# martius-lab/iCEM

Measured on AMD Instinct MI355X. Metric: traj-steps/sec (N x h), iCEM inner planning loop, higher is better.
Workload: dtype f32 storage; model step 2xfp16 planes (3 products), f32 accumulate

## Files before the change

icem_amd/_lib.py:

```python
from __future__ import annotations

import ctypes as C
import os

os.environ.setdefault("HSA_ENABLE_IPC_MODE_LEGACY", "0")
from typing import Optional

_HERE = os.path.dirname(os.path.abspath(__file__))
_LIB: Optional[C.CDLL] = None

ICEM_F32, ICEM_F64 = 0, 1
COST_MODES = {"sum": 0, "best": 1, "final": 2}
MODEL_LINEAR, MODEL_TANH = 0, 1
(BUF_MEAN, BUF_STD, BUF_LOW, BUF_HIGH, BUF_OBS0, BUF_ACTIONS, BUF_COSTS, BUF_ELITES, BUF_RECORDS,
 BUF_WORKSPACE, BUF_EXECUTED, BUF_BEST_COST, BUF_COUNT) = range(13)

KERNEL_NAMES = ["sample_clip", "rollout_cost", "topk_partial", "local_pack", "merge_refit", "sample_rollout"]

ICEM_E_INVALID, ICEM_E_UNSUPPORTED, ICEM_E_HIP, ICEM_E_NO_DEVICE, ICEM_E_STATE, ICEM_E_RANGE = -1, -2, -3, -4, -5, -6
ERR_NAMES = {-1: "ICEM_E_INVALID", -2: "ICEM_E_UNSUPPORTED", -3: "ICEM_E_HIP", -4: "ICEM_E_NO_DEVICE",
             -5: "ICEM_E_STATE", -6: "ICEM_E_RANGE"}


class IcemError(RuntimeError):
# ... 39 lines not shown
        "mean", "std", "low", "high", "obs0", "actions", "costs", "elites", "records", "workspace",
        "executed", "best_cost", "z_r", "z_i", "z_r_shift", "z_i_shift")]


_VP, _I32, _I64, _U64, _SZ = C.c_void_p, C.c_int32, C.c_int64, C.c_uint64, C.c_size_t
_H = C.c_void_p
SYMBOLS = [
    ("icem_abi_version", C.c_int, []),
    ("icem_build_hash", C.c_char_p, []),
    ("icem_last_error", C.c_char_p, []),
    ("icem_device_count", C.c_int, []),
    ("icem_create", C.c_int, [C.POINTER(IcemConfigC), C.POINTER(_H)]),
    ("icem_destroy", C.c_int, [_H]),
    ("icem_population_sizes", C.c_int, [_H, C.POINTER(_I32)]),
    ("icem_noise_tables_host", C.c_int, [_I32, C.c_double, C.POINTER(C.c_double), C.POINTER(C.c_double)]),
    ("icem_set_model", C.c_int, [_H, _I32, _I32, C.POINTER(C.c_double), C.POINTER(C.c_double)]),
    ("icem_set_cost", C.c_int, [_H, C.POINTER(IcemCostSpecC)]),
    ("icem_rssm_param_elems", _SZ, []),
    ("icem_rssm_rollout_cost", C.c_int, [_I32, _I32, _I32, _VP, _VP, _VP, _VP, _VP]),
    ("icem_rssm_rollout_cost_batch", C.c_int, [_I32, C.POINTER(_I32), _I32, _I32, _VP, _VP, _VP, _VP, _VP]),
    ("icem_get_action", C.c_int, [_H, C.POINTER(IcemPlanBuffersC), _I32, C.POINTER(C.c_double), C.POINTER(C.c_double),
                                  C.POINTER(C.c_double), _VP]),
    ("icem_set_cost_terms", C.c_int, [_H, C.POINTER(IcemCostTermsC)]),
    ("icem_trajectory_cost", C.c_int, [_H, _I32, _I32, _VP, _VP, _I64, _I64, _VP, _VP, _VP]),
    ("icem_sample_clip", C.c_int, [_H, _I32, _I64, _VP, _VP, _VP, _VP, _VP, _VP, _U64, _I32, _I32, _VP, _VP]),
    ("icem_sample_piecewise", C.c_int, [_H, _I32, _I64, _I32, _I64, _VP, _VP, _VP, _VP, _VP]),
    ("icem_philox_normals", C.c_int, [_H, _I32, _I64, _U64, _VP, _VP, _VP]),
    ("icem_rollout_cost", C.c_int, [_H, _I32, _VP, _VP, _VP, _VP, _VP]),
    ("icem_cost_reduce", C.c_int, [_H, _I32, _VP, _VP, _VP]),
    ("icem_topk_workspace_bytes", _SZ, [_H, _I32, _I32]),
    ("icem_topk_sorted", C.c_int, [_H, _I32, _VP, _I32, _VP, _VP, _VP, _VP]),
    ("icem_gather_refit", C.c_int, [_H, _VP, _VP, _I32, _VP, _VP, _VP, _VP]),
    ("icem_update_distribution", C.c_int, [_H, _I32, _VP, _VP, _I32, _VP, _VP, _I32, _VP, _VP, _VP, _VP, _VP, _VP]),
    ("icem_shift", C.c_int, [_H, _VP, _VP, _VP, _VP, _VP]),
    ("icem_reset_distribution", C.c_int, [_H, _VP, _VP, _VP, _VP, _VP]),
    ("icem_plan_buffer_bytes", _SZ, [_H, _I32]),
    ("icem_plan_iter_local", C.c_int, [_H, C.POINTER(IcemPlanBuffersC), _I32, _I32, _VP]),
    ("icem_plan_iter_merge", C.c_int, [_H, C.POINTER(IcemPlanBuffersC), _I32, _I32, _VP]),
    ("icem_plan_step", C.c_int, [_H, C.POINTER(IcemPlanBuffersC), _I32, _VP]),
    ("icem_record_bytes", _SZ, [_H]),
    ("icem_profile_enable", C.c_int, [_H, _I32]),
    ("icem_debug_stamps", C.c_int, [_H, _VP]),
    ("icem_set_merge_deferral", C.c_int, [_H, C.c_int32]),
    ("icem_set_episode", C.c_int, [_H, C.c_uint64]),
    ("icem_exchange_create", C.c_int, [_H, _VP]),
    ("icem_exchange_connect", C.c_int, [_H, _VP, C.POINTER(C.c_void_p)]),
    ("icem_exchange_block", C.c_void_p, [_H]),
    ("icem_exchange_disable", C.c_int, [_H]),
    ("icem_exchange_status", C.c_int, [_H, C.POINTER(C.c_int32), C.POINTER(C.c_int32)]),
    ("icem_plan_step_sharded", C.c_int, [_H, C.POINTER(IcemPlanBuffersC), _I32, _VP]),
    ("icem_exchange_probe", C.c_int, [_H, C.c_int32, _VP, C.POINTER(C.c_double)]),
    ("icem_sample_truncnorm", C.c_int, [_H, C.c_int32, C.c_int64, _VP, _VP, _VP, _VP, _VP, C.c_uint64, _VP, _VP]),
    ("icem_cem_bounds", C.c_int, [_H, C.c_int32, _VP, _VP, _VP, _VP, _VP, _VP, _VP]),
    ("icem_update_distribution_ok", C.c_int, [_H, C.c_int32, C.c_int32]),
    ("icem_rccl_load", C.c_int, [C.c_char_p]),
    ("icem_rccl_library", C.c_char_p, []),
    ("icem_rccl_unique_id", C.c_int, [_VP]),
    ("icem_rccl_connect", C.c_int, [_H, _VP]),
    ("icem_rccl_adopt", C.c_int, [_H, _VP]),
    ("icem_rccl_disconnect", C.c_int, [_H]),
    ("icem_allgather_elites", C.c_int, [_H, _VP, _VP]),
    ("icem_profile_read", C.c_int, [_H, C.POINTER(C.c_double), C.POINTER(C.c_int64), C.POINTER(C.c_int64)]),
    ("icem_rssm_trim", C.c_int, []),
    ("icem_set_wide_exact", C.c_int, [_H, _I32]),
    ("icem_set_wide_arith", C.c_int, [_H, _I32]),
    ("icem_wide_arith", C.c_int, [_H]),
    ("icem_wide_imbalance_log2", C.c_int, [_H]),
    ("icem_wide_model_imbalance_log2", C.c_int, [_I32, _I32, C.POINTER(C.c_double), C.POINTER(C.c_double)]),
    ("icem_set_tile_arith", C.c_int, [_H, _I32]),
    ("icem_tile_arith", C.c_int, [_H]),
    ("icem_set_f64_arith", C.c_int, [_H, _I32]),
    ("icem_f64_arith", C.c_int, [_H]),
    ("icem_profile_overhead", C.c_int, [_VP, _I32, C.c_double, C.POINTER(C.c_double), C.POINTER(C.c_double)]),
    ("icem_plan_step_batch", C.c_int, [C.POINTER(_H), _I32, C.POINTER(IcemPlanBuffersC), _I32, _VP]),
    ("icem_batch_uploads", C.c_int64, [_H]),
    ("icem_plan_step_batch_f64", C.c_int, [C.POINTER(_H), _I32, C.POINTER(IcemPlanBuffersC), _I32, _VP]),
    ("icem_batch_f64_launches", C.c_int64, [_H]),
    ("icem_plan_step_learned_ok", C.c_int, [_H]),
    ("icem_plan_step_learned", C.c_int, [_H, C.POINTER(IcemPlanBuffersC), _VP, _I32, _VP]),
    ("icem_plan_step_learned_batch", C.c_int, [C.POINTER(_H), _I32, C.POINTER(IcemPlanBuffersC), _VP, C.POINTER(_I32), _VP, _VP]),
    ("icem_learned_step_launches", C.c_int64, [_H]),
    ("icem_tile_growth", C.c_double, [_H]),
    ("icem_nonfinite_costs", C.c_int, [_H, C.POINTER(C.c_int64), _VP]),
    ("icem_set_option", C.c_int, [C.c_char_p, C.c_double]),
    ("icem_get_option", C.c_int, [C.c_char_p, C.POINTER(C.c_double)]),
    ("icem_reset_options", C.c_int, []),
    ("icem_option_name", C.c_char_p, [_I32]),
]


IPC_HANDLE_BYTES = 64
RCCL_ID_BYTES = 128
RSSM_OBS_DIM = 230
ABI_VERSION = 6


def lib_path() -> str:
    return os.environ.get("ICEM_HIP_LIB", os.path.join(_HERE, "libicem_hip.so"))


def load_library() -> C.CDLL:
    global _LIB
    if _LIB is not None:
        return _LIB
    path = lib_path()
    if not os.path.exists(path):
        raise ImportError(f"{path} not found: build it first (python -c 'import __graft_entry__ as g; g.build()'"
                          f" or python -m icem_amd.build)")
    lib = C.CDLL(path)
    for name, res, args in SYMBOLS:
        fn = getattr(lib, name)
        fn.restype = res
        fn.argtypes = args
    if lib.icem_abi_version() != ABI_VERSION:
        raise ImportError(f"{path}: ABI version {lib.icem_abi_version()} != {ABI_VERSION}: rebuild (python -m icem_amd.build)")
    _LIB = lib
    return lib


def option_names():
    lib = load_library()
    out, i = [], 0
    while True:
        n = lib.icem_option_name(i)
        if n is None:
            return out
        out.append(n.decode())
        i += 1


def set_option(name: str, value: float):
    check(load_library().icem_set_option(name.encode(), float(value)))


def get_option(name: str) -> float:
    v = C.c_double()
    check(load_library().icem_get_option(name.encode(), C.byref(v)))
    return v.value


def reset_options():
    check(load_library().icem_reset_options())


_ENV_WORDS = {"thread": 0.0, "rows": 1.0}


def apply_env_options(environ=None) -> dict:
    environ = os.environ if environ is None else environ
    done = {}
    for name in option_names():
        key = "ICEM_" + name.upper()
        if key in environ and environ[key] != "":
            raw = environ[key]
            val = _ENV_WORDS[raw] if raw in _ENV_WORDS else float(raw)
            set_option(name, val)
            done[name] = val
    if environ.get("ICEM_GK_ROLLOUT", "") == "thread":
        set_option("gk_rollout_thread", 1.0)
        done["gk_rollout_thread"] = 1.0
    return done


_FOLLOW_ENV = False


def follow_environment(on: bool = True):
    global _FOLLOW_ENV
    _FOLLOW_ENV = bool(on)
    if on:
        reset_options()
        apply_env_options()


def maybe_follow_environment():
    if _FOLLOW_ENV:
        reset_options()
        apply_env_options()


def check(rc: int):
    if rc != 0:
        msg = load_library().icem_last_error()
        raise IcemError(rc, msg.decode() if msg else "")
```

icem_amd/csrc/abi.hip:

```cpp
#include "host_common.h"
#include "cost_terms_dev.h"
#include "icem_rssm.h"

using namespace icem;

namespace {

void psd_scale_host(int h, double beta, std::vector<double>& s, double& sigma) {
    const int F = h / 2 + 1;
    s.resize(F);
    for (int k = 0; k < F; ++k) s[k] = (double)k * (1.0 / (double)h);
    const double fmin = 1.0 / (double)h;
    int ix = 0;
    for (int k = 0; k < F; ++k) ix += s[k] < fmin ? 1 : 0;
    if (ix && ix < F)
        for (int k = 0; k < ix; ++k) s[k] = s[ix];
    for (int k = 0; k < F; ++k) s[k] = std::pow(s[k], -beta / 2.0);
    double acc = 0.0;
    for (int k = 1; k < F; ++k) {
        double w = s[k];
        if (k == F - 1) w *= (1 + (h % 2)) / 2.0;
        acc += w * w;
    }
    sigma = 2.0 * std::sqrt(acc) / (double)h;
// ... 128 lines not shown
                                  "for its recurrence (that launch's costs are NaN); the staging flags were reset, nothing was "
                                  "launched by this call -- call again");
    ICEM_HIP_TRY(e);
    return ICEM_OK;
}

}

__global__ void profile_spin_kernel(long long ticks, long long* ran) {
    long long t0 = wall_clock64(), t = t0;
    for (long long polls = 0; t - t0 < ticks && polls < (1ll << 26); ++polls) t = wall_clock64();
    if (threadIdx.x == 0) *ran = t - t0;
}

extern "C" {

int icem_abi_version(void) { return ICEM_ABI_VERSION; }

#ifndef ICEM_BUILD_HASH
#define ICEM_BUILD_HASH "0000000000000000"
#endif
const char* icem_build_hash(void) {
    static const char tag[] = "ICEM_BUILD_HASH=" ICEM_BUILD_HASH;
    return tag + 16;
}

const char* icem_last_error(void) { return g_err.c_str(); }

int icem_device_count(void) {
    int n = 0;
    if (hipGetDeviceCount(&n) != hipSuccess) return 0;
    return n;
}

int icem_noise_tables_host(int32_t horizon, double beta, double* cr_host, double* ci_host) {
    if (horizon < 2 || !cr_host || !ci_host) return fail(ICEM_E_INVALID, "bad horizon / null output");
    std::vector<double> cr, ci;
    noise_tables(horizon, beta, cr, ci);
    std::memcpy(cr_host, cr.data(), cr.size() * sizeof(double));
    std::memcpy(ci_host, ci.data(), ci.size() * sizeof(double));
    return ICEM_OK;
}

int icem_create(const icem_config* cfg, icem_handle** out) {
    if (!cfg || !out) return fail(ICEM_E_INVALID, "null argument");
    const icem_config& c = *cfg;
    if (c.num_traj < 2) return fail(ICEM_E_INVALID, "At least two trajectories needed!");
    if (c.horizon < 2 || c.horizon > ICEM_MAX_HORIZON) return fail(ICEM_E_UNSUPPORTED, "horizon must be in [2, 64]");
    if (c.act_dim < 1 || c.act_dim > ICEM_MAX_ACT_DIM) return fail(ICEM_E_UNSUPPORTED, "act_dim must be in [1, 64]");
    if (c.num_elites < 1 || c.num_elites > ICEM_MAX_ELITES) return fail(ICEM_E_UNSUPPORTED, "num_elites must be in [1, 64]");
    if (c.opt_iters < 1) return fail(ICEM_E_INVALID, "opt_iters < 1");
    if (c.dtype != ICEM_F32 && c.dtype != ICEM_F64) return fail(ICEM_E_INVALID, "dtype");
    if (c.rng_rounds != 10 && c.rng_rounds != 7) return fail(ICEM_E_INVALID, "rng_rounds must be 10 or 7");
    if (c.world < 1 || c.rank < 0 || c.rank >= c.world) return fail(ICEM_E_INVALID, "rank/world");
    if (c.noise_beta != c.noise_beta) return fail(ICEM_E_INVALID, "noise_beta is NaN");
    if (!(c.factor_decrease >= 1.0)) return fail(ICEM_E_INVALID, "factor_decrease must be >= 1");
    if (c.cost_mode < 0 || c.cost_mode > 2)
        return fail(ICEM_E_UNSUPPORTED, "Implement method to compute cost along trajectory");
    if (icem_device_count() < 1) return fail(ICEM_E_NO_DEVICE, "no HIP device visible");
    icem_handle* h = new icem_handle();
    h->cfg = c;
    h->F = c.horizon / 2 + 1;
    h->HMAX = c.horizon <= 32 ? 32 : 64;
    h->hd = c.horizon * c.act_dim;
    h->tsize = c.dtype == ICEM_F64 ? 8 : 4;
    h->pop = population_sizes(c);
    h->n_reuse = (int)((double)c.num_elites * c.fraction_reused);
    h->n_local_max = 0;
    for (int n_it : h->pop) h->n_local_max = std::max(h->n_local_max, shard_chunk(n_it, c.world));
    h->use_fast = opt_i(OPT_DISABLE_FAST) == 0;
    std::vector<double> cr, ci, W((size_t)c.horizon * h->HMAX, 0.0);
    if (c.noise_beta > 0) {
        noise_tables(c.horizon, c.noise_beta, cr, ci);
        for (int t = 0; t < c.horizon; ++t)
            for (int m = 0; m < c.horizon; ++m)
                W[(size_t)t * h->HMAX + m] = m < h->F ? cr[(size_t)m * c.horizon + t] : ci[(size_t)(m - h->F + 1) * c.horizon + t];
    } else {
        for (int t = 0; t < c.horizon; ++t) W[(size_t)t * h->HMAX + t] = 1.0;
    }
    int rc = c.dtype == ICEM_F64 ? upload<double>(&h->W_dev, W) : upload<float>(&h->W_dev, W);
    if (!rc && (hipMalloc((void**)&h->nonfinite_dev, 2 * sizeof(unsigned)) != hipSuccess ||
                hipMemset(h->nonfinite_dev, 0, 2 * sizeof(unsigned)) != hipSuccess))
        rc = fail(ICEM_E_HIP, "hipMalloc of the handle's status word failed");
    if (rc) {
        if (h->W_dev) (void)hipFree(h->W_dev);
        if (h->nonfinite_dev) (void)hipFree(h->nonfinite_dev);
        delete h;
        return rc;
    }
    *out = h;
    return ICEM_OK;
}

int icem_destroy(icem_handle* h) {
    if (!h) return ICEM_OK;
    xchg_destroy(h);
    rccl_release(h);
    ahead_destroy(h);
    if (h->W_dev) (void)hipFree(h->W_dev);
    if (h->nonfinite_dev) (void)hipFree(h->nonfinite_dev);
    if (h->actions_alt) (void)hipFree(h->actions_alt);
    if (h->host_stage) (void)hipHostFree(h->host_stage);
    if (h->ws_alt) (void)hipFree(h->ws_alt);
    if (h->pp_stats) (void)hipFree(h->pp_stats);
    if (h->A_dev) (void)hipFree(h->A_dev);
    if (h->B_dev) (void)hipFree(h->B_dev);
    if (h->Mp_dev) (void)hipFree(h->Mp_dev);
    if (h->Mw_dev) (void)hipFree(h->Mw_dev);
    if (h->Mws_dev) (void)hipFree(h->Mws_dev);
    if (h->Mwh_dev) (void)hipFree(h->Mwh_dev);
    if (h->Mwh_ksc_dev) (void)hipFree(h->Mwh_ksc_dev);
    if (h->wide_cs_dev) (void)hipFree(h->wide_cs_dev);
    if (h->M64_dev) (void)hipFree(h->M64_dev);
    if (h->f64_cs_dev) (void)hipFree(h->f64_cs_dev);
    if (h->hn_cs_dev) (void)hipFree(h->hn_cs_dev);
    if (h->pub_dev) (void)hipFree(h->pub_dev);
    if (h->perm_dev) (void)hipFree(h->perm_dev);
    for (auto& sp : h->spans) {
        (void)hipEventDestroy(sp.a);
        (void)hipEventDestroy(sp.b);
    }
    for (auto e : h->free_events) (void)hipEventDestroy(e);
    delete h;
    return ICEM_OK;
}

int icem_set_episode(icem_handle* h, uint64_t episode) {
    if (check_handle(h)) return ICEM_E_INVALID;
    if (episode >> 32) return fail(ICEM_E_INVALID, "episode must fit 32 bits");
    h->episode = episode;
    return ICEM_OK;
}

int icem_population_sizes(const icem_handle* h, int32_t* out_host) {
    if (!h || !out_host) return fail(ICEM_E_INVALID, "null argument");
    for (size_t i = 0; i < h->pop.size(); ++i) out_host[i] = h->pop[i];
    return ICEM_OK;
}

static void update_paths(icem_handle* h) {
    const bool tile = !h->wide && h->has_model && !h->has_terms && !(h->has_cost && h->cost.lin_weight == 0.0) &&
                      fast_rollout_supported(h->cfg.horizon, h->cfg.act_dim, h->O, 1);
    const int of = tile ? h->O : 0;
    if (of != h->Of) h->fast_model_ready = false;
    h->Of = of;
    bool split_ok = of >= 16 && of <= 20 && h->cfg.dtype == ICEM_F32 && !(h->cost.flip_idx >= 0 && h->cost.flip_thresh < 0.0);
    auto lift = [](const std::vector<double>& m, bool* finite) {
        double mx = 0.0;
        for (double v : m) {
            mx = std::max(mx, std::fabs(v));
            if (!(std::fabs(v) < 1e30)) *finite = false;
        }
        if (!(mx > 1e-30)) return 1.f;
        int e = 0;
        (void)std::frexp(mx, &e);
        return (float)std::ldexp(1.0, 7 - e);
    };
    bool finite = true;
    h->tile_m_scale = lift(h->A_host, &finite);
    h->tile_b_scale = lift(h->B_host, &finite);
    const bool narrow_f32 = !h->wide && h->has_model && h->cfg.dtype == ICEM_F32 && finite;
    const bool hn_shape = h->has_model && h->cfg.dtype == ICEM_F32 && finite && h->obs_dim <= 48;
    h->tile_growth = 1.0;
    h->tile_ratio_log2 = 0;
    if ((narrow_f32 || hn_shape) && !h->A_host.empty()) {
        if (h->model_kind == ICEM_MODEL_LINEAR)
            h->tile_growth = linear_growth_bound(h->obs_dim, h->cfg.act_dim, h->cfg.horizon, h->A_host, h->B_host);
        int ea = 0, eb = 0;
        (void)std::frexp((double)h->tile_m_scale, &ea);
        (void)std::frexp((double)h->tile_b_scale, &eb);
        double bmax = 0.0;
        for (double v : h->B_host) bmax = std::max(bmax, std::fabs(v));
        h->tile_ratio_log2 = bmax > 1e-30 ? ea - eb : 0;
    }
    const bool range_ok = finite && h->tile_growth <= 1024.0 && h->tile_ratio_log2 <= 10;
    split_ok = split_ok && range_ok;
    const int mode = h->tile_arith_mode;
    const bool want = mode == 1 || mode < 0;
    h->tile_arith = (split_ok && want) ? 1 : 0;
    int n32 = 0, n4 = 0, np = 0;
    bool terms_ok = true;
    if (h->has_terms && (h->terms.diff_idx >= 0 || h->terms.health_idx >= 0)) terms_ok = false;
    if (h->has_terms)
// ... 1 lines not shown
            const icem_cost_term& tm = h->terms.terms[j];
            if (tm.kind == ICEM_TERM_STEP_GT || tm.kind == ICEM_TERM_SQ_OFFSET) ++np;
            else if (tm.len <= 4) ++n4;
            else if (tm.len <= 32) ++n32;
            else terms_ok = false;
        }
    int prog[3] = {0, 0, 0};
    const bool hn = of == 0 && h->has_model && h->has_cost && h->cfg.dtype == ICEM_F32 && range_ok && mode != 0 && terms_ok &&
                    !(h->wide && h->wide_mode == ICEM_WIDE_F32) &&
                    hn_cost_program(n32, n4, np, prog) &&
                    hn_rollout_supported(h->cfg.horizon, h->cfg.act_dim, h->obs_dim, h->cfg.num_elites);
    for (int k = 0; k < 3; ++k) h->hn_prog[k] = hn ? prog[k] : 0;
    if (hn != h->hn_tile) h->fast_model_ready = false;
    h->hn_tile = hn;
    int eff = 0;
    if (h->wide && h->has_model) {
        eff = h->wide_mode >= 0 ? h->wide_mode : (h->wide_imbalance > 13 ? 2 : 0);
        if (!wide_split_fits(h->obs_dim, h->cfg.act_dim)) eff = 1;
    } else if (gemm_rollout(h)) {
        eff = 1;
    }
    if (eff != h->wide_eff) h->fast_model_ready = false;
    h->wide_eff = eff;
}

static int sync_wide_cost(icem_handle* h);
static int sync_f64_mfma(icem_handle* h);

int icem_set_tile_arith(icem_handle* h, int32_t mode) {
    if (check_handle(h)) return ICEM_E_INVALID;
    if (mode < -1 || mode > 1) return fail(ICEM_E_INVALID, "tile arithmetic: -1 (by configuration), 0 (exact f32) or 1 (fp16 planes)");
    if (h->ride.merge_pending || h->ride.pack_pending) return fail(ICEM_E_STATE, "a deferred merge is pending: finish the MPC step first");
    h->tile_arith_mode = mode;
    update_paths(h);
    h->ahead.next_valid = h->ahead.pre_valid = false;
    return sync_wide_cost(h);
}

int icem_tile_arith(const icem_handle* h) { return h ? ((h->tile_arith || h->hn_tile) ? 1 : 0) : 0; }

double icem_tile_growth(const icem_handle* h) { return h ? h->tile_growth : 0.0; }

int icem_set_option(const char* name, double value) {
    if (!name || !(value == value)) return fail(ICEM_E_INVALID, "null option name / NaN value");
    for (int k = 0; k < OPT_COUNT; ++k)
        if (std::strcmp(name, OPT_ROWS[k].name) == 0) {
            g_opt[k].store(value, std::memory_order_relaxed);
            return ICEM_OK;
        }
    return fail(ICEM_E_INVALID, std::string("unknown option: ") + name);
}

int icem_get_option(const char* name, double* value_out) {
    if (!name || !value_out) return fail(ICEM_E_INVALID, "null argument");
    for (int k = 0; k < OPT_COUNT; ++k)
        if (std::strcmp(name, OPT_ROWS[k].name) == 0) {
            *value_out = g_opt[k].load(std::memory_order_relaxed);
            return ICEM_OK;
        }
    return fail(ICEM_E_INVALID, std::string("unknown option: ") + name);
}

int icem_reset_options(void) {
    for (int k = 0; k < OPT_COUNT; ++k) g_opt[k].store(OPT_ROWS[k].def, std::memory_order_relaxed);
    return ICEM_OK;
}

const char* icem_option_name(int32_t index) { return (index >= 0 && index < OPT_COUNT) ? OPT_ROWS[index].name : nullptr; }

int icem_nonfinite_costs(icem_handle* h, int64_t* count_out, void* stream) {
    if (check_handle(h)) return ICEM_E_INVALID;
    if (!count_out) return fail(ICEM_E_INVALID, "null output");
    hipStream_t st = (hipStream_t)stream;
    hipStreamCaptureStatus cap = hipStreamCaptureStatusNone;
    if (hipStreamIsCapturing(st, &cap) == hipSuccess && cap != hipStreamCaptureStatusNone)
        return fail(ICEM_E_STATE, "icem_nonfinite_costs synchronises: not on a capturing stream");
    unsigned v = 0;
    ICEM_HIP_TRY(hipMemcpyAsync(&v, h->nonfinite_dev, sizeof(v), hipMemcpyDeviceToHost, st));
    ICEM_HIP_TRY(hipStreamSynchronize(st));
    *count_out = (int64_t)v;
    return ICEM_OK;
}

int icem_set_model(icem_handle* h, int32_t kind, int32_t obs_dim, const double* A_host, const double* B_host) {
    if (!h || !A_host || !B_host) return fail(ICEM_E_INVALID, "null argument");
    if (kind != ICEM_MODEL_LINEAR && kind != ICEM_MODEL_TANH) return fail(ICEM_E_INVALID, "model kind");
    const int d = h->cfg.act_dim;
    if (obs_dim > 32 && h->cfg.dtype == ICEM_F64 && h->f64_arith == ICEM_F64_MFMA) {
        if (obs_dim > ICEM_MAX_OBS_DIM || f64_mfma_lds_bytes(obs_dim, d) > 160 * 1024)
            return fail(ICEM_E_UNSUPPORTED, "obs_dim must be in [1, 384]");
        if (h->A_dev) (void)hipFree(h->A_dev);
        if (h->B_dev) (void)hipFree(h->B_dev);
        h->A_dev = h->B_dev = nullptr;
        h->model_kind = kind;
        h->obs_dim = obs_dim;
        h->O = 0;
        h->wide = false;
        h->has_model = true;
        h->A_host.assign(A_host, A_host + (size_t)obs_dim * obs_dim);
        h->B_host.assign(B_host, B_host + (size_t)d * obs_dim);
        h->fast_model_ready = false;
        h->f64_model_ready = false;
        update_paths(h);
        return sync_wide_cost(h);
    }
    if (obs_dim > 32) {
        if (h->cfg.dtype != ICEM_F32 || !wide_rollout_supported(obs_dim, d, 1))
            return fail(ICEM_E_UNSUPPORTED, "obs_dim in (32, 384] needs dtype f32 (k_rollout_wide) or, on an f64 handle, "
                                            "icem_set_f64_arith(ICEM_F64_MFMA); beyond 384 is not compiled");
        if (h->cfg.num_elites > 32) return fail(ICEM_E_UNSUPPORTED, "obs_dim > 32 needs num_elites <= 32 (candidate lists of k_rollout_wide)");
        if (h->A_dev) (void)hipFree(h->A_dev);
        if (h->B_dev) (void)hipFree(h->B_dev);
        h->A_dev = h->B_dev = nullptr;
        h->model_kind = kind;
        h->obs_dim = obs_dim;
        h->O = 0;
        h->wide = true;
        h->has_model = true;
        h->A_host.assign(A_host, A_host + (size_t)obs_dim * obs_dim);
        h->B_host.assign(B_host, B_host + (size_t)d * obs_dim);
        h->wide_imbalance = wide_model_imbalance_log2(obs_dim, d, h->A_host.data(), h->B_host.data());
        h->fast_model_ready = false;
        update_paths(h);
        return sync_wide_cost(h);
    }
    const int O = pick_O(obs_dim);
    if (obs_dim < 1 || O < 0) return fail(ICEM_E_UNSUPPORTED, "obs_dim must be in [1, 384]");
    h->wide = false;
    std::vector<double> A((size_t)O * O, 0.0), B((size_t)d * O, 0.0);
    for (int k = 0; k < obs_dim; ++k)
        for (int i = 0; i < obs_dim; ++i) A[(size_t)k * O + i] = A_host[(size_t)k * obs_dim + i];
    for (int j = 0; j < d; ++j)
        for (int i = 0; i < obs_dim; ++i) B[(size_t)j * O + i] = B_host[(size_t)j * obs_dim + i];
    int rc = h->cfg.dtype == ICEM_F64 ? upload<double>(&h->A_dev, A) : upload<float>(&h->A_dev, A);
    if (rc) return rc;
    rc = h->cfg.dtype == ICEM_F64 ? upload<double>(&h->B_dev, B) : upload<float>(&h->B_dev, B);
    if (rc) return rc;
    h->model_kind = kind;
    h->obs_dim = obs_dim;
    h->O = O;
    h->has_model = true;
    h->A_host.assign(A_host, A_host + (size_t)obs_dim * obs_dim);
    h->B_host.assign(B_host, B_host + (size_t)d * obs_dim);
    h->fast_model_ready = false;
    h->f64_model_ready = false;
    update_paths(h);
    return sync_wide_cost(h);
}

static int sync_f64_mfma(icem_handle* h) {
    if (h->cfg.dtype != ICEM_F64 || h->f64_arith != ICEM_F64_MFMA) return ICEM_OK;
    if (h->has_model && !h->f64_model_ready) {
        const int o = h->obs_dim, d = h->cfg.act_dim, Op = (o + 15) & ~15, Kp = (o + d + 3) & ~3;
        std::vector<double> M((size_t)Kp * Op, 0.0);
        for (int k = 0; k < o; ++k)
            for (int i = 0; i < o; ++i) M[(size_t)k * Op + i] = h->A_host[(size_t)k * o + i];
        for (int j = 0; j < d; ++j)
            for (int i = 0; i < o; ++i) M[(size_t)(o + j) * Op + i] = h->B_host[(size_t)j * o + i];
        const int rc = upload<double>(&h->M64_dev, M);
        if (rc) return rc;
        h->f64_model_ready = true;
    }
    if (h->has_cost) {
        CostArgs<double> cs;
        std::memset((void*)&cs, 0, sizeof(cs));
        fill_cost_args_f64(h, cs);
// ... 367 lines not shown
```

icem_amd/csrc/fused_dev.h:

```cpp
#pragma once
#include "icem_fused.h"

#include <climits>
#include <cmath>
#include <cstdlib>
#include <algorithm>
#include <type_traits>
#include <utility>

#include "exchange_dev.h"
#include "philox.h"
#include "refit.h"

#ifndef ICEM_FAST_SHAPES
#define ICEM_FAST_SHAPES(X) X(30, 6, 17) X(30, 6, 18) X(12, 6, 17) X(13, 4, 17) X(30, 17, 24)
#endif
#define ICEM_FAST_HORIZONS(X) X(30) X(12) X(13) X(10)

namespace icem {

namespace {

constexpr int HMAX = 32;
constexpr int SWG = 256;
// ... 886 lines not shown
        use_min = a.cost_mode == 1;
        flip_th = a.flip_th;
    }
    __device__ __forceinline__ void load_obs(const float* obs) {
        x_init = obs[perm_c];
#pragma unroll
        for (int r = 0; r < REM; ++r) rem_init[r] = obs[perm_rem[r]];
    }
    __device__ __forceinline__ const float* read_ptr(const float* buf, int row, int stride) const {
        return buf + T16::SLACK + row * stride + (g - REM);
    }
    __device__ __forceinline__ const float* row_ptr(const float* buf, int row, int stride) const {
        return buf + T16::SLACK + row * stride;
    }
    struct State {
        float x;
        float xr[REM > 0 ? REM : 1];
        float acc_s, acc_b;
    };
    __device__ __forceinline__ void init(State& st) const {
        st.x = x_init;
#pragma unroll
        for (int r = 0; r < REM; ++r) st.xr[r] = rem_init[r];
        st.acc_s = 0.f;
        st.acc_b = INFINITY;
    }
    __device__ __forceinline__ void step(State& st, const float* rd, const float* ar) const {
        float xv[NKX];
#pragma unroll
        for (int q = 0; q < NKX; ++q) {
            const float ld = rd[4 * q];
            float v = is_act[q] ? ld : 0.f;
#pragma unroll
            for (int r = 0; r < REM; ++r)
                if (r / 4 == q) v = (g == r % 4) ? st.xr[r] : v;
            xv[q] = v;
        }
        float ext[NE];
#pragma unroll
        for (int e = 0; e < NE; ++e) ext[e] = e < REM ? st.xr[e] : (e - REM < D ? ar[e - REM] : 0.f);
        const float col0 = dpp_f32<0x00>(st.x);
        const float col1 = dpp_f32<0x55>(st.x);
        const float ang = ang_is_col1 ? col1 : col0;
        float cst = 0.f;
        cst += (ang > flip_th) ? pen : 0.f;
        cst += (ang < -flip_th) ? pen : 0.f;
#pragma unroll
        for (int q = 0; q < NKX; ++q) cst = __builtin_fmaf(xv[q] * xv[q], cw[q], cst);
        cst = __builtin_fmaf(lin_w, col0, cst);
        float pr[REM > 0 ? REM : 1];
        if (REM > 0) {
            const float col2 = dpp_f32<0xAA>(st.x), col3 = dpp_f32<0xFF>(st.x);
            const float cq[4] = {col0, col1, col2, col3};
#pragma unroll
            for (int r = 0; r < REM; ++r) {
                float p = 0.f;
#pragma unroll
                for (int s = 0; s < 4; ++s) p = __builtin_fmaf(cq[s], wq[r][s], p);
#pragma unroll
                for (int q = 0; q < NKX; ++q) p = __builtin_fmaf(xv[q], wx[r][q], p);
                pr[r] = reduce_quads(p);
            }
        }
        cst = reduce_quads(cst);
        st.acc_s = __builtin_fmaf(st.acc_s, ksum, cst);
        st.acc_b = cst < st.acc_b ? cst : st.acc_b;
        float nxt = 0.f;
        asm volatile("s_nop 1" ::: "memory");
#define ICEM_T4(K) nxt = fmac_row_bcast<K>(nxt, st.x, mK[K]);
        ICEM_T4(0) ICEM_T4(4) ICEM_T4(8) ICEM_T4(12)
        ICEM_T4(1) ICEM_T4(5) ICEM_T4(9) ICEM_T4(13)
        ICEM_T4(2) ICEM_T4(6) ICEM_T4(10) ICEM_T4(14)
        ICEM_T4(3) ICEM_T4(7) ICEM_T4(11) ICEM_T4(15)
#undef ICEM_T4
#pragma unroll
        for (int e = 0; e < NE; ++e) nxt = __builtin_fmaf(mE[e], ext[e], nxt);
        st.x = act_fn(nxt, std::integral_constant<int, KIND>{});
#pragma unroll
        for (int r = 0; r < REM; ++r) st.xr[r] = act_fn(pr[r], std::integral_constant<int, KIND>{});
    }
    __device__ __forceinline__ float cost(const State& st) const { return use_min ? st.acc_b : st.acc_s; }
};

template <bool LANE_MASK = true>
__device__ __forceinline__ unsigned long long topk_push16(unsigned long long run_key, unsigned long long key, bool first,
                                                          int K, int lane) {
    if (!first) {
        const unsigned long long prev = __shfl(run_key, lane - 16, 64);
        if (lane >= 16 && lane < 16 + K) key = prev;
    }
    return wave_sort_n<LANE_MASK>(key, lane, first ? 16u : 16u + (unsigned)K);
}

constexpr unsigned KEY_FILL_LO = 0x7FFFFE00u;
template <int WAVES>
__device__ __forceinline__ void wg_merge_emit(unsigned long long (*wg_keys)[WAVES][32], unsigned long long run_key, int K,
                                              int lane, int wave, const FastRolloutArgs& a, int wg = blockIdx.x,
                                              int n_wg = gridDim.x) {
    static_assert(WAVES * 32 <= 512, "filler keys: one per slot");
    auto emit = [&](unsigned long long key, int place) {
        if (a.part_k) {
            a.part_k[(size_t)place * n_wg + wg] = key;
        } else {
            a.part_c[(size_t)wg * K + place] = key_cost(key);
            a.part_i[(size_t)wg * K + place] = key_idx(key);
        }
    };
    if (WAVES == 1) {
        if (wave == 0 && lane < K) emit(run_key, lane);
        return;
    }
    const int kp = (K + 1) & ~1, half = kp >> 1;
    unsigned long long* keys = &wg_keys[0][0][0];
    if (wave < WAVES && lane < kp) {
        unsigned long long v = lane < K ? run_key : KEY_SENTINEL;
        if (v == KEY_SENTINEL) v = (KEY_SENTINEL & 0xFFFFFFFF00000000ull) | (KEY_FILL_LO + (unsigned)(wave * 32 + lane));
        keys[wave * 32 + lane] = v;
    }
    __syncthreads();
    if (wave < WAVES) {
        const int q = lane >> 4;
        for (int s0 = 0; s0 < K; s0 += 16) {
            const int i = s0 + (lane & 15);
            const unsigned long long mine = keys[wave * 32 + (i < 32 ? i : 31)];
            unsigned place = 0;
            for (int r = q; r < WAVES; r += 4) {
                const unsigned long long* b = keys + r * 32;
#pragma unroll 4
                for (int c = 0; c < half; ++c) place += (b[2 * c] < mine ? 1u : 0u) + (b[2 * c + 1] < mine ? 1u : 0u);
            }
            place += (unsigned)__shfl_xor((int)place, 16, 64);
            place += (unsigned)__shfl_xor((int)place, 32, 64);
            if (q == 0 && i < K && place < (unsigned)K) {
                const bool filler = (mine >> 32) == (KEY_SENTINEL >> 32) && (unsigned)mine >= KEY_FILL_LO;
                emit(filler ? KEY_SENTINEL : mine, (int)place);
            }
        }
    }
}

constexpr int MERGE_WG = 256;
constexpr int LPL = 4;

template <int CTRL, int ROW_MASK>
__device__ __forceinline__ unsigned long long min_dpp(unsigned long long x) {
    const int lo = __builtin_amdgcn_update_dpp((int)(unsigned)x, (int)(unsigned)x, CTRL, ROW_MASK, 0xF, false);
    const int hi = __builtin_amdgcn_update_dpp((int)(unsigned)(x >> 32), (int)(unsigned)(x >> 32), CTRL, ROW_MASK, 0xF, false);
    const unsigned long long o = ((unsigned long long)(unsigned)hi << 32) | (unsigned)lo;
    return o < x ? o : x;
}

__device__ __forceinline__ unsigned long long wave_min_u64(unsigned long long x) {
    x = min_dpp<0xB1, 0xF>(x);
    x = min_dpp<0x4E, 0xF>(x);
    x = min_dpp<0x141, 0xF>(x);
    x = min_dpp<0x140, 0xF>(x);
    x = min_dpp<0x142, 0xA>(x);
    x = min_dpp<0x143, 0xC>(x);
    const unsigned lo = __builtin_amdgcn_readlane((int)(unsigned)x, 63);
    const unsigned hi = __builtin_amdgcn_readlane((int)(unsigned)(x >> 32), 63);
    return ((unsigned long long)hi << 32) | lo;
}

template <int CTRL, int ROW_MASK>
__device__ __forceinline__ unsigned min_dpp32(unsigned x) {
    const unsigned o = (unsigned)__builtin_amdgcn_update_dpp((int)x, (int)x, CTRL, ROW_MASK, 0xF, false);
    return o < x ? o : x;
}
__device__ __forceinline__ unsigned wave_min_u32(unsigned x) {
    x = min_dpp32<0xB1, 0xF>(x);
    x = min_dpp32<0x4E, 0xF>(x);
    x = min_dpp32<0x141, 0xF>(x);
    x = min_dpp32<0x140, 0xF>(x);
    x = min_dpp32<0x142, 0xA>(x);
    x = min_dpp32<0x143, 0xC>(x);
    return (unsigned)__builtin_amdgcn_readlane((int)x, 63);
}
__device__ __forceinline__ unsigned long long wave_min_key(unsigned long long x) {
    const unsigned hi = (unsigned)(x >> 32), lo = (unsigned)x;
    const unsigned mh = wave_min_u32(hi);
    const unsigned long long tie = __ballot(hi == mh);
    unsigned ml;
    if (__popcll(tie) == 1)
        ml = (unsigned)__builtin_amdgcn_readlane((int)lo, __ffsll((long long)tie) - 1);
    else
        ml = wave_min_u32(hi == mh ? lo : 0xFFFFFFFFu);
    return ((unsigned long long)mh << 32) | ml;
}

template <int CTRL, int ROW_MASK>
__device__ __forceinline__ unsigned add_dpp(unsigned x) {
    return x + (unsigned)__builtin_amdgcn_update_dpp(0, (int)x, CTRL, ROW_MASK, 0xF, ROW_MASK == 0xF);
}
__device__ __forceinline__ unsigned wave_incl_scan_u32(unsigned x) {
    x = add_dpp<0x111, 0xF>(x);
    x = add_dpp<0x112, 0xF>(x);
    x = add_dpp<0x114, 0xF>(x);
    x = add_dpp<0x118, 0xF>(x);
    x = add_dpp<0x142, 0xA>(x);
    x = add_dpp<0x143, 0xC>(x);
    return x;
}

__device__ __forceinline__ unsigned long long lds_reread_u64(const unsigned long long* p) {
#ifdef ICEM_DEBUG
    if (!__builtin_amdgcn_is_shared(p)) __builtin_trap();
#endif
    return *(const volatile __attribute__((address_space(3))) unsigned long long*)p;
}

__device__ __forceinline__ int keep_index0(const MergeSingleArgs& a) { return a.keep_base >= 0 ? a.keep_base : a.n_global; }

__device__ __forceinline__ float merge_keep_cost(const MergeSingleArgs& a, int lane) {
    const bool has = a.elites_cost_cur != nullptr;
    const float* src = has ? a.elites_cost_cur : reinterpret_cast<const float*>(a.part_k);
    const float v = src[(has && lane < a.n_keep) ? lane : 0];
    return has ? v : 0.f;
}

template <int KREG>
__device__ __forceinline__ void merge_select(const MergeSingleArgs& a, int lane, unsigned long long* cand,
                                             unsigned long long* sel) {
    unsigned long long k[LPL][KREG];
    const float keep_cost = merge_keep_cost(a, lane);
#pragma unroll
    for (int l = 0; l < LPL; ++l) {
        const int list = lane + l * 64;
#pragma unroll
        for (int i = 0; i < KREG; ++i)
            k[l][i] = a.part_k[(size_t)(i < a.K ? i : 0) * a.n_lists + (list < a.n_lists ? list : 0)];
    }
#pragma unroll
    for (int l = 0; l < LPL; ++l) {
        const bool has_list = lane + l * 64 < a.n_lists;
#pragma unroll
        for (int i = 0; i < KREG; ++i) k[l][i] = (has_list && i < a.K) ? k[l][i] : KEY_SENTINEL;
    }
    if (a.dbg && threadIdx.x == 0) a.dbg[1] = wall_clock64();
    if (lane < a.n_keep) {
        unsigned long long v = make_key(keep_cost, keep_index0(a) + lane);
#pragma unroll
        for (int i = 0; i < KREG; ++i) {
            const bool sw = v < k[0][i];
            const unsigned long long t = sw ? k[0][i] : v;
            k[0][i] = sw ? v : k[0][i];
            v = t;
        }
    }
    if (a.dbg && threadIdx.x == 0) a.dbg[2] = wall_clock64();
    unsigned long long mine = k[0][0];
#pragma unroll
    for (int l = 1; l < LPL; ++l) mine = k[l][0] < mine ? k[l][0] : mine;
    const unsigned srt = wave_sort64_u32((unsigned)(mine >> 32), lane);
    const unsigned T = __shfl(srt, a.K - 1, 64);
    unsigned n_cand = 0;
#pragma unroll
    for (int i = 0; i < KREG; ++i) {
        bool p[LPL];
        bool any_lane = false;
#pragma unroll
        for (int l = 0; l < LPL; ++l) {
            p[l] = (unsigned)(k[l][i] >> 32) <= T && k[l][i] != KEY_SENTINEL;
            any_lane |= p[l];
        }
        if (__ballot(any_lane) == 0) break;
#pragma unroll
        for (int l = 0; l < LPL; ++l) {
            const unsigned long long m = __ballot(p[l]);
            if (m != 0) {
                const unsigned pos = n_cand + __builtin_amdgcn_mbcnt_hi((unsigned)(m >> 32), __builtin_amdgcn_mbcnt_lo((unsigned)m, 0u));
                if (p[l] && pos < 64) cand[pos] = k[l][i];
                n_cand += (unsigned)__popcll(m);
            }
        }
    }
    if (a.dbg && threadIdx.x == 0) a.dbg[3] = wall_clock64();
    __builtin_amdgcn_fence(__ATOMIC_SEQ_CST, "workgroup");
    if (n_cand <= 64) {
        unsigned long long key = lane < (int)n_cand ? lds_reread_u64(&cand[lane]) : KEY_SENTINEL;
        key = wave_sort_n(key, lane, n_cand);
        if (lane < a.K) sel[lane] = key;
    } else {
        for (int r = 0; r < a.K; ++r) {
            unsigned long long head = k[0][0];
#pragma unroll
            for (int l = 1; l < LPL; ++l) head = k[l][0] < head ? k[l][0] : head;
            const unsigned long long best = wave_min_u64(head);
            if (best != KEY_SENTINEL) {
#pragma unroll
                for (int l = 0; l < LPL; ++l) {
                    if (k[l][0] == best) {
#pragma unroll
                        for (int i = 0; i + 1 < KREG; ++i) k[l][i] = k[l][i + 1];
                        k[l][KREG - 1] = KEY_SENTINEL;
                    }
                }
            }
            if (lane == 0) sel[r] = best;
        }
    }
}

__device__ __forceinline__ void merge_select_stream(const MergeSingleArgs& a, int lane, unsigned long long* cand,
                                                    unsigned long long* sel) {
    const int K = a.K, nl = a.n_lists;
    auto key_at = [&](int l, int i) -> unsigned long long {
        const int list = lane + l * 64;
        const unsigned long long v = a.part_k[(size_t)(i < K ? i : 0) * nl + (list < nl ? list : 0)];
        return (list < nl && i < K) ? v : KEY_SENTINEL;
    };
    const unsigned long long kept = lane < a.n_keep ? make_key(a.elites_cost_cur[lane], keep_index0(a) + lane) : KEY_SENTINEL;
    unsigned long long mine = kept;
#pragma unroll
    for (int l = 0; l < LPL; ++l) {
        const unsigned long long v = key_at(l, 0);
        mine = v < mine ? v : mine;
    }
    const unsigned long long srt = wave_sort64(mine, lane);
    const unsigned long long T = __shfl(srt, K - 1, 64);
    unsigned n_cand = 0;
    auto offer = [&](unsigned long long key) {
        const bool p = key <= T && key != KEY_SENTINEL;
        const unsigned long long m = __ballot(p);
        if (m != 0) {
            const unsigned pos = n_cand + __builtin_amdgcn_mbcnt_hi((unsigned)(m >> 32), __builtin_amdgcn_mbcnt_lo((unsigned)m, 0u));
            if (p && pos < 64) cand[pos] = key;
            n_cand += (unsigned)__popcll(m);
        }
        return m != 0;
    };
    offer(kept);
#pragma unroll 1
    for (int l = 0; l < LPL; ++l) {
        if (l * 64 >= nl) break;
#pragma unroll 1
        for (int i = 0; i < K; ++i)
            if (!offer(key_at(l, i))) break;
    }
    __builtin_amdgcn_fence(__ATOMIC_SEQ_CST, "workgroup");
    if (n_cand <= 64) {
        unsigned long long key = lane < (int)n_cand ? lds_reread_u64(&cand[lane]) : KEY_SENTINEL;
        key = wave_sort_n(key, lane, n_cand);
        if (lane < K) sel[lane] = key;
    } else {
        int cur[LPL];
#pragma unroll
        for (int l = 0; l < LPL; ++l) cur[l] = 0;
        bool kept_live = true;
        for (int r = 0; r < K; ++r) {
            unsigned long long head = kept_live ? kept : KEY_SENTINEL;
#pragma unroll
            for (int l = 0; l < LPL; ++l) {
                const unsigned long long v = key_at(l, cur[l]);
                head = v < head ? v : head;
            }
            const unsigned long long best = wave_min_u64(head);
            if (best != KEY_SENTINEL) {
                if (kept_live && kept == best) kept_live = false;
#pragma unroll
                for (int l = 0; l < LPL; ++l)
                    if (key_at(l, cur[l]) == best) ++cur[l];
            }
            if (lane == 0) sel[r] = best;
        }
    }
}

template <int DEPTH>
__device__ __forceinline__ void merge_select_shallow(const MergeSingleArgs& a, int lane, unsigned long long* cand,
                                                     unsigned long long* sel) {
    const int K = a.K, nl = a.n_lists;
    const float keep_cost = merge_keep_cost(a, lane);
    unsigned long long k[LPL][DEPTH];
#pragma unroll
    for (int l = 0; l < LPL; ++l) {
        const int list = lane + l * 64;
#pragma unroll
        for (int i = 0; i < DEPTH; ++i) k[l][i] = a.part_k[(size_t)(i < K ? i : 0) * nl + (list < nl ? list : 0)];
    }
#pragma unroll
    for (int l = 0; l < LPL; ++l) {
        const bool has_list = lane + l * 64 < nl;
#pragma unroll
        for (int i = 0; i < DEPTH; ++i) k[l][i] = (has_list && i < K) ? k[l][i] : KEY_SENTINEL;
    }
    const unsigned long long kept = lane < a.n_keep ? make_key(keep_cost, keep_index0(a) + lane) : KEY_SENTINEL;
    unsigned long long mine = k[0][0];
#pragma unroll
    for (int l = 1; l < LPL; ++l) mine = k[l][0] < mine ? k[l][0] : mine;
    const unsigned srt = wave_sort64_u32((unsigned)(mine >> 32), lane);
    const unsigned T = __shfl(srt, K - 1, 64);
    unsigned n_cand = 0;
    auto offer = [&](unsigned long long key) {
        const bool p = (unsigned)(key >> 32) <= T && key != KEY_SENTINEL;
        const unsigned long long m = __ballot(p);
        if (m != 0) {
            const unsigned pos = n_cand + __builtin_amdgcn_mbcnt_hi((unsigned)(m >> 32), __builtin_amdgcn_mbcnt_lo((unsigned)m, 0u));
            if (p && pos < 64) cand[pos] = key;
            n_cand += (unsigned)__popcll(m);
        }
        return m != 0;
    };
    bool deeper[LPL];
#pragma unroll
    for (int l = 0; l < LPL; ++l) {
        deeper[l] = true;
#pragma unroll
        for (int i = 0; i < DEPTH; ++i)
            if (deeper[l]) deeper[l] = offer(k[l][i]);
    }
#pragma unroll 1
    for (int l = 0; l < LPL; ++l) {
        if (!deeper[l]) continue;
#pragma unroll 1
        for (int i = DEPTH; i < K; ++i) {
            const int list = lane + l * 64;
            const unsigned long long v = list < nl ? a.part_k[(size_t)i * nl + list] : KEY_SENTINEL;
            if (!offer(v)) break;
        }
    }
    offer(kept);
    __builtin_amdgcn_fence(__ATOMIC_SEQ_CST, "workgroup");
    if (n_cand <= 64) {
        unsigned long long key = lane < (int)n_cand ? lds_reread_u64(&cand[lane]) : KEY_SENTINEL;
        key = wave_sort_n(key, lane, n_cand);
        if (lane < K) sel[lane] = key;
    } else {
        merge_select_stream(a, lane, cand, sel);
    }
}

__device__ __forceinline__ void merge_select_records(const MergeSingleArgs& a, int lane, unsigned long long* cand,
                                                     unsigned long long* sel, int* slot, long long* stamp = nullptr) {
    const int K = a.K, rs = a.h * a.d + 2;
    xchg_wait(a.xw, lane);
    if (stamp && lane == 0) *stamp = wall_clock64();
    auto rec_key = [&](int e) -> unsigned long long {
        if (e >= a.n_rec) return KEY_SENTINEL;
        const float* rec = a.records + (size_t)e * rs;
        return make_key(rec[0], reinterpret_cast<const int*>(rec + 1)[0]);
    };
    unsigned long long k[3] = {rec_key(lane), rec_key(lane + 64),
                               lane < a.n_keep ? make_key(a.elites_cost_cur[lane], a.n_global + lane) : KEY_SENTINEL};
    const unsigned long long k0 = k[0], k1 = k[1], k2 = k[2];
    for (int r = 0; r < K; ++r) {
        unsigned long long head = k[0] < k[1] ? k[0] : k[1];
        head = k[2] < head ? k[2] : head;
        const unsigned long long best = wave_min_key(head);
        if (best != KEY_SENTINEL) {
            if (k0 == best) { slot[r] = lane; k[0] = KEY_SENTINEL; }
            if (k1 == best) { slot[r] = lane + 64; k[1] = KEY_SENTINEL; }
            if (k2 == best) { slot[r] = a.n_rec + lane; k[2] = KEY_SENTINEL; }
        } else if (lane == 0) {
            slot[r] = 0;
        }
        if (lane == 0) sel[r] = best;
    }
    (void)cand;
}

__device__ __forceinline__ void merge_select_records_wg(const MergeSingleArgs& a, bool stager, int lane, int tid, int nthr,
                                                        unsigned long long* sel, int* slot, long long* stamp = nullptr) {
    __shared__ unsigned long long rk_keys[192];
    __shared__ unsigned rk_rank[192];
    const int K = a.K, rs = a.h * a.d + 2;
    if (stager) {
        xchg_wait(a.xw, lane);
        if (stamp && lane == 0) *stamp = wall_clock64();
        auto rec_key = [&](int e) -> unsigned long long {
            if (e >= a.n_rec) return KEY_SENTINEL;
            const float* rec = a.records + (size_t)e * rs;
            return make_key(rec[0], reinterpret_cast<const int*>(rec + 1)[0]);
        };
        rk_keys[lane] = rec_key(lane);
        rk_keys[64 + lane] = rec_key(lane + 64);
        rk_keys[128 + lane] = lane < a.n_keep ? make_key(a.elites_cost_cur[lane], a.n_global + lane) : KEY_SENTINEL;
        rk_rank[lane] = rk_rank[64 + lane] = rk_rank[128 + lane] = 0u;
        sel[lane] = KEY_SENTINEL;
        slot[lane] = 0;
    }
    __syncthreads();
    const int n_rec = a.n_rec, n_live = n_rec + a.n_keep;
    auto at = [&](int c) { return c < n_rec ? c : 128 + (c - n_rec); };
    int parts = n_live > 0 ? nthr / n_live : 1;
    parts = parts < 1 ? 1 : (parts > 8 ? 8 : parts);
    if (n_live > 0 && tid < n_live * parts) {
        const int c = tid % n_live, p = tid / n_live;
        const unsigned long long mine = rk_keys[at(c)];
        unsigned cnt = 0;
        for (int j = p; j < n_live; j += parts) cnt += rk_keys[at(j)] < mine ? 1u : 0u;
        if (cnt) atomicAdd(&rk_rank[at(c)], cnt);
    }
    if (n_live > nthr)
        for (int c = nthr + tid; c < n_live; c += nthr) {
            const unsigned long long mine = rk_keys[at(c)];
            unsigned cnt = 0;
            for (int j = 0; j < n_live; ++j) cnt += rk_keys[at(j)] < mine ? 1u : 0u;
            rk_rank[at(c)] = cnt;
        }
    __syncthreads();
    for (int c = tid; c < n_live; c += nthr) {
        const unsigned long long mine = rk_keys[at(c)];
        const unsigned r = rk_rank[at(c)];
        if (mine != KEY_SENTINEL && r < (unsigned)K) {
            sel[r] = mine;
            slot[r] = c;
        }
    }
    __syncthreads();
}

// ... 477 lines not shown
```

icem_amd/csrc/host_common.h:

```cpp
#pragma once
#include <hip/hip_runtime.h>

#include <cfloat>
#include <climits>
#include <cmath>
#include <cstdio>
#include <cstdlib>
#include <cstring>
#include <algorithm>
#include <atomic>
#include <string>
#include <type_traits>
#include <vector>

#include "../../include/icem_hip.h"
#include "arg_array.h"
#include "icem_fused.h"
#include "options.h"

namespace icem {

inline thread_local std::string g_err;

inline int fail(int code, const std::string& msg) {
    g_err = msg;
    return code;
}

#define ICEM_HIP_TRY(expr)                                                                      \
    do {                                                                                        \
        hipError_t e_ = (expr);                                                                 \
        if (e_ != hipSuccess)                                                                   \
            return ::icem::fail(ICEM_E_HIP, std::string(#expr) + ": " + hipGetErrorString(e_)); \
    } while (0)

constexpr int WG = 256;
constexpr int TOPK_CHUNK = 1024;

struct Exchange;

struct LearnedCtx {
    DeviceArgArray<2> args;
    float* pool = nullptr;
    size_t pool_rows = 0;
    int pool_n = 0;
    int* idx = nullptr;
    long long launches = 0;
    ~LearnedCtx() {
        if (pool) (void)hipFree(pool);
        if (idx) (void)hipFree(idx);
    }
};

}

struct icem_handle {
    icem_config cfg;
    int F = 0, HMAX = 0, hd = 0;
    size_t tsize = 4;
    void* W_dev = nullptr;
    int model_kind = 0, obs_dim = 0, O = 0;
    void* A_dev = nullptr;
    void* B_dev = nullptr;
    bool has_model = false, has_cost = false;
    icem_cost_spec cost;
    icem_cost_terms terms;
    bool has_terms = false;
    void* host_stage = nullptr;
    void* host_stage_dev = nullptr;
    unsigned io_seq = 0;
    std::vector<int> pop;
    int n_reuse = 0;
    int n_local_max = 0;
    bool profiling = false;
    struct Span {
        int kind;
        long long units;
        hipEvent_t a, b;
    };
    bool use_fast = true;
    long long* dbg = nullptr;
    struct LocalReport {
        int lists = 0;
        int tail_rows = 0;
        int sel_cand = 0, sel_loc = 0;
        void clear() { *this = LocalReport(); }
    } local;
    void* actions_alt = nullptr;
    void* ws_alt = nullptr;
    float* pp_stats = nullptr;
    struct Riding {
        bool merge_pending = false;
        icem::MergeSingleArgs merge;
        bool pack_pending = false;
        icem::PackPrev pack;
        void clear() { merge_pending = pack_pending = false; }
    } ride;
    bool deferral = false;
    float* cur_mean = nullptr;
    float* cur_std = nullptr;
    bool wide = false;
    int Of = 0;
    int tile_arith_mode = -1;
    int tile_arith = 0;
    int hn_prog[3] = {0, 0, 0};
    void* hn_cs_dev = nullptr;
    bool hn_tile = false;
    float tile_m_scale = 1.f, tile_b_scale = 1.f;
    float act_mag = 1.f;
    const void* am_lo = nullptr;
    const void* am_hi = nullptr;
    double tile_growth = 1.0;
    int tile_ratio_log2 = 0;
    unsigned* nonfinite_dev = nullptr;
    unsigned nonfinite_seen = 0;
    void* Mw_dev = nullptr;
    void* Mws_dev = nullptr;
    void* Mwh_dev = nullptr;
    float Mwh_inv = 1.f;
    void* Mwh_ksc_dev = nullptr;
    int Mwh_nk = 0;
    float Mwh_sbound = 0.f;
    int wide_mode = -1;
    int wide_eff = 0;
    int wide_imbalance = 0;
    int wide_packed = -2;
    void* wide_cs_dev = nullptr;
    int f64_arith = 0;
    void* M64_dev = nullptr;
    bool f64_model_ready = false;
    void* f64_cs_dev = nullptr;
    void* Mp_dev = nullptr;
    void* perm_dev = nullptr;
    int flip_col = -1;
    bool fast_model_ready = false;
    std::vector<double> A_host, B_host;
    std::vector<Span> spans;
    std::vector<hipEvent_t> free_events;
    icem::Exchange* xchg = nullptr;
    icem::XchgWait xw_last;
    uint64_t episode = 0;
    float* pub_dev = nullptr;
    unsigned pub_seq = 0;
    struct Ahead {
        void* pool[3] = {nullptr, nullptr, nullptr};
        unsigned long long ctr = 0;
        bool next_valid = false;
        uint64_t next_episode = 0;
        int next_step = -1;
        void* next_pool = nullptr;
        hipStream_t next_stream = nullptr;
        const void* lo_ptr = nullptr;
        const void* hi_ptr = nullptr;
        bool uniform = false;
        float lo = 0.f, hi = 0.f;
        bool tail_pending = false;
        icem::FastSampleArgs tail_args, tail2_args;
        int next1_rows = 0;
        void* next1_pool = nullptr;
        void* pre_raw = nullptr;
        bool pre_valid = false;
        uint64_t pre_episode = 0;
        int pre_step = -1;
        hipStream_t pre_stream = nullptr;
        int disabled = -1;
        int min_rows = 0;
    } ahead;
    icem::DeviceArgArray<6> batch_args;
    unsigned long long batch_uploads = 0;
    long long batch_f64_launches = 0;
    icem::LearnedCtx learned;
    void* rccl_comm = nullptr;
    bool rccl_owned = false;
};

namespace icem {

struct ProfScope {
    icem_handle* h;
    hipStream_t st;
    hipEvent_t a = nullptr, b = nullptr;
    int kind;
    long long units;
    static hipEvent_t get(icem_handle* h) {
        if (!h->free_events.empty()) {
            hipEvent_t e = h->free_events.back();
            h->free_events.pop_back();
            return e;
        }
        hipEvent_t e = nullptr;
        (void)hipEventCreate(&e);
        return e;
    }
    ProfScope(const icem_handle* hc, int kind_, long long units_, hipStream_t st_)
        : h(const_cast<icem_handle*>(hc)), st(st_), kind(kind_), units(units_) {
        if (!h->profiling) return;
        a = get(h);
        b = get(h);
// ... 151 lines not shown
```

icem_amd/csrc/icem_fused.h:

```cpp
#pragma once
#include <hip/hip_runtime.h>
#include <stdint.h>
#include <cstddef>
#include <cstring>
#include <vector>
#include "cost_args.h"
#include "options.h"

namespace icem {

constexpr int FAST_MAX_LISTS = 256;
struct BatchHint;
struct LaunchCtx;

constexpr int XCHG_MAX_WORLD = 16;
struct XchgWait {
    const unsigned* flags = nullptr;
    unsigned* status = nullptr;
    unsigned seq = 0;
    int world = 0;
    unsigned max_polls = 0;
    const void* records = nullptr;
};
struct XchgPush {
// ... 160 lines not shown
    const float* keep_actions;
    int n, n_keep, K, hd;
    float alpha;
    float* mean;
    float* std;
    float* elites_out;
    float* elite_costs_out;
    int* idx_out;
};
void launch_update_small(const UpdateSmallArgs& a, hipStream_t st);
constexpr int UPDATE_FINISH_MAX_HD = 256;
struct UpdateFinishArgs {
    UpdateSmallArgs u;
    int d;
    float init_std;
    const float* low;
    const float* high;
    float* executed;
    float* best_cost;
    float* result;
};
void launch_update_small_batch(const UpdateFinishArgs* args_dev, int n, bool finish, hipStream_t st);
bool topk_small_ok(int n, int K);
void launch_topk_small(const float* costs, int n, int K, float* out_c, int* out_i, hipStream_t st);
bool pack_can_push(int K, int h, int d);
void launch_pack_records(const MergeSingleArgs& a, int n_loc, int shard_lo, float* records, hipStream_t st,
                         const XchgPush& px = XchgPush());
void launch_pack_merge(const MergeSingleArgs& pk, int n_loc, int shard_lo, float* records, const XchgPush& px, const MergeSingleArgs& m,
                       hipStream_t st);

struct PackPrev {
    const unsigned long long* part_k = nullptr;
    const float* actions = nullptr;
    int n_lists = 0, n_pool = 0, n_global = 0, K = 0;
    int n_loc = 0, shard_lo = 0;
    int n_keep = 0;
    const float* keep_costs = nullptr;
    float* records = nullptr;
    XchgPush px;
    float* pub = nullptr;
    unsigned* pub_flag = nullptr;
    unsigned pub_seq = 0;
};
bool sample_rollout_pack_ok(const BatchHint& bh, int h, int d, int O, int rounds, int n_rows, int K);
bool sample_folded_pack_ok(int h, int d, int rounds, int K);

void launch_noise_rows(const FastSampleArgs& a, int rounds, hipStream_t st);
struct IterAheadArgs {
    FastRolloutArgs r;
    MergeSingleArgs m;
    int has_merge;
    int n_xf;
    int row0_mean;
    int store_back;
    float* pool;
    const float* mean;
    const float* std;
    float lo, hi;
    FastSampleArgs z;
    FastSampleArgs s;
    PackPrev p;
    int n_roll, n_noise;
    int dbg_slot = 0;
};
bool rollout_ahead_ok(const BatchHint& bh, int h, int d, int O, int K, int n_rows);
int ahead_roll_workgroups(const BatchHint& bh, int n_rows);
void launch_iter_ahead(const LaunchCtx& cx, const IterAheadArgs& a, int h, int d, int O, int kind);

struct FastSampleMergeArgs {
    FastSampleArgs s;
    MergeSingleArgs m;
    PackPrev p;
};
bool sample_folded_merge_ok(int h, int d, int rounds, int K);
void launch_sample_folded_merge(const LaunchCtx& cx, const FastSampleMergeArgs& a);
bool sample_batch_compiled(int h);

struct FastIterArgs {
    FastSampleArgs s;
    FastRolloutArgs r;
    MergeSingleArgs m;
    PackPrev p;
};
}
#include "generic_args.h"
namespace icem {
constexpr int ICEM_MAX_BATCH = 32;
struct BatchBases {
    unsigned long long v[ICEM_MAX_BATCH];
};
struct BatchHint {
    int mult = 1;
    bool ahead = false;
};
enum LaunchFamily : int { LAUNCH_SAMPLE_ROLLOUT = 1, LAUNCH_ITER_AHEAD = 2, LAUNCH_MERGE_NOISE = 3, LAUNCH_SAMPLE = 4, LAUNCH_SAMPLE_MERGE = 5,
                          LAUNCH_ROLLOUT_HN = 6, LAUNCH_GK_SAMPLE = 7, LAUNCH_GK_SHIFT = 8, LAUNCH_GK_ROLLOUT_ROWS = 9, LAUNCH_GK_ROLLOUT_THREAD = 10,
                          LAUNCH_GK_SELECT = 11, LAUNCH_ROLLOUT_WIDE = 12, LAUNCH_ROLLOUT_WIDE_SPLIT = 13, LAUNCH_ROLLOUT_ROWS_WIDE = 14 };
struct LaunchKey {
    int family = 0;
    int h = 0, d = 0, O = 0, kind = 0, arith = 0;
    int waves = 0;
    int form = 0;
    int wgs[3] = {0, 0, 0};
    bool operator==(const LaunchKey& o) const { return std::memcmp(this, &o, sizeof(LaunchKey)) == 0; }
};
struct MergeNoiseBatchArgs {
    MergeSingleArgs a;
    FastSampleArgs z1, z2;
};
struct LaunchDesc {
    LaunchKey key;
    static constexpr size_t BLOCK = sizeof(IterAheadArgs) > sizeof(RolloutArgs<double>) ? sizeof(IterAheadArgs) : sizeof(RolloutArgs<double>);
    static_assert(sizeof(SelectArgs<double>) <= BLOCK && sizeof(SampleArgs<double>) <= BLOCK, "LaunchDesc::block");
    alignas(8) unsigned char block[BLOCK];
};
struct LaunchRecorder {
    unsigned long long base = 0;
    std::vector<LaunchDesc> launches;
    bool unsupported = false;
    const char* who = "icem_plan_step_batch: ";
    void* add(const LaunchKey& key) {
        launches.emplace_back();
        launches.back().key = key;
        std::memset(launches.back().block, 0, sizeof(launches.back().block));
        return launches.back().block;
    }
};
struct LaunchCtx {
    hipStream_t st = nullptr;
    BatchHint hint;
    LaunchRecorder* rec = nullptr;
};
template <class Form, class Issue>
void submit(const LaunchCtx& cx, const LaunchKey& key, bool batched_form, Form&& form, Issue&& issue) {
    if (!cx.rec) return issue();
    if (!batched_form) cx.rec->unsupported = true;
    else form(cx.rec->add(key), cx.rec->base);
}
inline void sub_base(uint32_t& lo, uint32_t& hi, unsigned long long base) {
    const unsigned long long v = (((unsigned long long)hi << 32) | lo) - base;
    lo = (uint32_t)v;
    hi = (uint32_t)(v >> 32);
}
inline void batch_form(const FastIterArgs& a, unsigned long long base, void* dst) {
    std::memcpy(dst, &a, sizeof(a));
    FastSampleArgs& s = ((FastIterArgs*)dst)->s;
    if (s.n_shift == 0) s.off2_lo = s.off2_hi = 0;
    else sub_base(s.off2_lo, s.off2_hi, base);
    sub_base(s.off_lo, s.off_hi, base);
}
inline void batch_form(const IterAheadArgs& a, unsigned long long base, void* dst) {
    constexpr size_t defined = offsetof(IterAheadArgs, dbg_slot) + sizeof(int);
    std::memcpy(dst, &a, defined);
    IterAheadArgs& g = *(IterAheadArgs*)dst;
    g.r.dbg = nullptr;
    if (g.z.n > 0) sub_base(g.z.off_lo, g.z.off_hi, base);
    else g.z.off_lo = g.z.off_hi = 0;
    if (g.s.n_shift > 0) {
        sub_base(g.s.off_lo, g.s.off_hi, base);
        sub_base(g.s.off2_lo, g.s.off2_hi, base);
    } else {
        g.s.off_lo = g.s.off_hi = g.s.off2_lo = g.s.off2_hi = 0;
    }
}
inline void batch_form(const MergeSingleArgs& a, const FastSampleArgs* z1, const FastSampleArgs* z2, unsigned long long base, void* dst) {
    MergeNoiseBatchArgs& g = *(MergeNoiseBatchArgs*)dst;
// ... 139 lines not shown
```

icem_amd/csrc/k_iter_small.hip:

```cpp
#include "fused_dev.h"

namespace icem {

namespace {

constexpr bool sr_quad(int d, int rw) { return rw <= 2 && ((4 * 16 * rw * d + 63) / 64) * 64 + 64 <= 1024; }
constexpr int sr_threads(int d, int rw) { return (((sr_quad(d, rw) ? 4 : 1) * 16 * rw * d + 63) / 64) * 64; }

template <int H, int D, int O, int KIND, int ROUNDS, int RW, int KREG, bool REC, int ARITH>
__device__ __forceinline__ void sample_rollout_body(const FastSampleArgs& sa, const FastRolloutArgs& ra, const MergeSingleArgs& am,
                                                    const PackPrev& ap) {
    constexpr bool PM = KREG > 0;
    constexpr bool QS = sr_quad(D, RW);
    constexpr bool T4 = QS && O <= 20 && sr_threads(D, RW) >= 256 * RW && ARITH == 0;
    using T16 = typename TileSel<H, D, O, KIND, ARITH>::type;
    using Tile = typename std::conditional<T4, Tile4<H, D, (O <= 20 ? O : 17), KIND>, T16>::type;
    constexpr int RWV = T4 ? 4 * RW : RW;
    constexpr int HD = H * D;
    constexpr int TPB = 16 * RW;
    constexpr int ROWS = TPB * D;
    constexpr int NT = sr_threads(D, RW);
    constexpr int NTT = NT + (PM ? 64 : 0);
    static_assert(NTT <= 1024 && HD % 2 == 0, "workgroup shape");
    constexpr int VW = HD % 4 == 0 ? 4 : 2;
    using Vec = typename VecOf<VW>::type;
    __shared__ __attribute__((aligned(16))) float ms[2 * HD];
    __shared__ __attribute__((aligned(16))) float tilebuf[T16::SLACK + TPB * HD + T16::TAIL];
    __shared__ unsigned long long wg_keys[2][RW][32];
    __shared__ float obs_stage[32];
    constexpr int WROWS = H / 2 + 1;
    __shared__ __attribute__((aligned(16))) float Wl[QS ? NT / 64 : 1][QS ? WROWS * WQ_STRIDE : 4];
    __shared__ unsigned long long sel[PM ? 64 : 1];
    __shared__ unsigned long long cand[PM ? 64 : 1];
    __shared__ int slot[PM ? 64 : 1];
    float* tile_rows = tilebuf + T16::SLACK;
    const int tid = threadIdx.x;
    const int lane = tid & 63;
    const int wave = tid >> 6;
    const int n_rows = ra.n_rows;
    const bool has_pack = PM && REC && ap.part_k != nullptr;
    if constexpr (PM && REC) {
        if (has_pack && blockIdx.x == 0) {
            MergeSingleArgs pk{};
            pk.n_lists = ap.n_lists;
            pk.n_pool = ap.n_pool;
            pk.n_global = ap.n_global;
            pk.K = ap.K;
            pk.h = H;
            pk.d = D;
            pk.part_k = ap.part_k;
            pk.actions = ap.actions;
            pk.n_keep = ap.n_keep;
            pk.elites_cost_cur = ap.keep_costs;
            pk.keep_base = ap.n_loc;
            __builtin_amdgcn_s_setprio(3);
            if (ra.dbg && tid == 0) ra.dbg[0] = wall_clock64();
            if (tid < 64) {
                if constexpr (NTT <= 512)
                    merge_select<12>(pk, lane, cand, sel);
                else
                    merge_select_stream(pk, lane, cand, sel);
            }
            __syncthreads();
            if (ra.dbg && tid == 0) ra.dbg[1] = wall_clock64();
            pack_records_body<12>(pk, ap.n_loc, ap.shard_lo, ap.records, ap.px, tilebuf, sel, tid, NTT);
            if (ra.dbg && tid == 0) ra.dbg[2] = wall_clock64();
            return;
        }
    }
    const int wg = blockIdx.x - (has_pack ? 1 : 0);
    const int n_wg = ra.list_wgs > 0 ? ra.list_wgs : (int)gridDim.x - (has_pack ? 1 : 0);
    const int base = wg * TPB;
    if (base >= n_rows) return;
    if (ra.dbg && tid == 0 && wg == 0) ra.dbg[8] = wall_clock64();
    const int rowi = QS ? tid >> 2 : tid, q = tid & 3;
    const int nl = rowi / D, jd = rowi - nl * D;
    const bool has_row = rowi < ROWS;
    float* trow = tile_rows + nl * HD + jd;
    const float* mrow = ms + jd;
    Tile tile;
    float obs_reg = 0.f;
    constexpr int WPL = (WROWS * HMAX + 63) / 64;
    float wreg[QS ? WPL : 1];
    const bool pre_drawn = !PM && sa.raw_src != nullptr;
    if constexpr (QS) {
        if (tid < NT && !pre_drawn) {
#pragma unroll
            for (int i = 0; i < WPL; ++i) wreg[i] = sa.W[(i * 64 + lane) < WROWS * HMAX ? i * 64 + lane : 0];
        }
    }
    const int r_mine = base + nl;
    float lo_reg = 0.f, hi_reg = 0.f;
    if ((PM || pre_drawn) && tid < NT) {
        lo_reg = sa.low[jd];
        hi_reg = sa.high[jd];
    }
    constexpr int NVR = !PM ? (TPB * (HD / VW) + NTT - 1) / NTT : 1;
    constexpr int NVB = NVR < 4 ? NVR : 4;
    constexpr int NEL = !PM && QS ? (H - 1 + 3) / 4 : 1;
    typedef float RawV __attribute__((ext_vector_type(VW)));
    RawV rawv[NVB];
    float elv[NEL];
    if (!PM) {
        const int total4 = (n_rows - base < TPB ? n_rows - base : TPB) * (HD / VW);
        RawV* t4 = reinterpret_cast<RawV*>(tile_rows);
        float mreg[(HD + NTT - 1) / NTT], sreg[(HD + NTT - 1) / NTT];
#pragma unroll
        for (int i = 0; i < (HD + NTT - 1) / NTT; ++i) {
            const int e = tid + i * NTT;
            mreg[i] = sa.mean[e < HD ? e : 0];
            sreg[i] = sa.std[e < HD ? e : 0];
        }
        if (pre_drawn) {
            const RawV* g4 = reinterpret_cast<const RawV*>(sa.raw_src + (size_t)base * HD);
#pragma unroll
            for (int i = 0; i < NVB; ++i) {
                const int e = tid + i * NTT;
                rawv[i] = g4[e < total4 ? e : 0];
            }
            if constexpr (QS) {
                if (has_row && tid < NT && r_mine >= sa.n && r_mine < n_rows) {
                    const float* src = sa.elites_src + (size_t)(r_mine - sa.n) * HD + jd;
#pragma unroll
                    for (int i = 0; i < NEL; ++i) elv[i] = src[(q + 4 * i < H - 1 ? q + 4 * i + 1 : 1) * D];
                }
            }
        }
        obs_reg = ra.obs0[(tid < 32 && tid < ra.o) ? tid : 0];
        if (wave < RWV) tile.load(ra, lane);
#pragma unroll
        for (int i = 0; i < (HD + NTT - 1) / NTT; ++i) {
            const int e = tid + i * NTT;
            if (e < HD) {
                ms[e] = mreg[i];
                ms[HD + e] = sreg[i];
            }
        }
        if (pre_drawn) {
#pragma unroll
            for (int i = 0; i < NVB; ++i) {
                const int e = tid + i * NTT;
                if (e < total4) t4[e] = rawv[i];
            }
            if constexpr (NVR > NVB) {
                const RawV* g4 = reinterpret_cast<const RawV*>(sa.raw_src + (size_t)base * HD);
                for (int e0 = tid + NVB * NTT; e0 < total4; e0 += NVB * NTT) {
#pragma unroll
                    for (int i = 0; i < NVB; ++i) rawv[i] = g4[e0 + i * NTT < total4 ? e0 + i * NTT : 0];
#pragma unroll
                    for (int i = 0; i < NVB; ++i)
                        if (e0 + i * NTT < total4) t4[e0 + i * NTT] = rawv[i];
                }
            }
        }
// ... 4 lines not shown
        if (has_row && tid < NT) {
            const float lo = lo_reg, hi = hi_reg;
            constexpr int QN = QS ? 4 : 1;
            const int q0 = QS ? q : 0;
            if (r_mine < sa.n) {
                for (int t = q0; t < H; t += QN) {
                    const float v = __builtin_fmaf(trow[t * D], mrow[HD + t * D], mrow[t * D]);
                    trow[t * D] = __builtin_amdgcn_fmed3f(v, lo, hi);
                }
            } else if (r_mine < n_rows) {
                const float* src = sa.elites_src + (size_t)(r_mine - sa.n) * HD + jd;
                if ((H - 1) % QN == q0) {
                    const float v = __builtin_fmaf(trow[(H - 1) * D], mrow[HD + (H - 1) * D], mrow[(H - 1) * D]);
                    trow[(H - 1) * D] = __builtin_amdgcn_fmed3f(v, lo, hi);
                }
                if constexpr (QS) {
#pragma unroll
                    for (int i = 0; i < NEL; ++i)
                        if (q + 4 * i < H - 1) trow[(q + 4 * i) * D] = elv[i];
                } else {
                    for (int t = q0; t < H - 1; t += QN) trow[t * D] = src[(t + 1) * D];
                }
            } else {
                for (int t = q0; t < H; t += QN) trow[t * D] = 0.f;
            }
        }
    } else
    if constexpr (QS) {
        if (tid < NT) {
            float* wl = Wl[wave];
            sample_into_tile_quad<H, D, ROUNDS, PM>(sa, has_row, n_rows, r_mine, jd, q, trow, mrow, wl, [&]() {
#pragma unroll
                for (int i = 0; i < WPL; ++i) {
                    const int e = i * 64 + lane;
                    if (e < WROWS * HMAX) wl[(e / HMAX) * WQ_STRIDE + (e % HMAX)] = wreg[i];
                }
                __builtin_amdgcn_fence(__ATOMIC_RELEASE, "wavefront");
                __builtin_amdgcn_wave_barrier();
                __builtin_amdgcn_fence(__ATOMIC_ACQUIRE, "wavefront");
            });
        }
    } else if (has_row) {
        sample_into_tile<H, D, ROUNDS, PM>(sa, n_rows, r_mine, jd, trow, mrow);
    }
    if constexpr (PM) {
        if (tid >= NT) {
            if constexpr (RW <= 4) __builtin_amdgcn_s_setprio(3);
            if constexpr (REC) {
                if (ra.dbg && lane == 0 && wg == 0) ra.dbg[3] = wall_clock64();
            }
            else if constexpr (RW >= 8)
                merge_select_stream(am, lane, cand, sel);
            else
                merge_select_shallow<3>(am, lane, cand, sel);
        }
    }
    if (PM) {
        obs_reg = ra.obs0[(tid < 32 && tid < ra.o) ? tid : 0];
        if (wave < RWV) tile.load(ra, lane);
    }
    const float* rd0 = nullptr;
    if constexpr (!T4) rd0 = tile.read_ptr(tilebuf + (wave < RW ? wave : 0) * 16 * HD, lane, HD);
    if constexpr (PM) {
        const MergeSingleArgs& m = am;
        if constexpr (REC) {
            merge_select_records_wg(am, tid >= NT, lane, tid, NTT, sel, slot, (ra.dbg && wg == 0) ? ra.dbg + 7 : nullptr);
            if (ra.dbg && tid == 0 && wg == 0) ra.dbg[4] = wall_clock64();
        } else {
            __syncthreads();
        }
        if (ra.dbg && tid == 0 && wg == 0) ra.dbg[5] = wall_clock64();
        if (!REC && ra.dbg && tid == 0 && wg == 0) ra.dbg[15] = wall_clock64();
        const float* rows[KREG > 0 ? KREG : 1];
        merge_rows<KREG, REC>(m, sel, slot, rows);
        for (int e = tid; e < HD; e += NTT) {
            float xs[KREG > 0 ? KREG : 1];
#pragma unroll
            for (int r = 0; r < KREG; ++r) xs[r] = rows[r][e];
            float nm, ns;
            refit_element_regs<float, KREG>(m.K, m.alpha, m.mean[e], m.std[e], xs, nm, ns);
            ms[e] = nm;
            ms[HD + e] = ns;
            if (wg == 0) {
                m.mean_out[e] = nm;
                m.std_out[e] = ns;
#pragma unroll
                for (int r = 0; r < KREG; ++r)
                    if (r < m.K) m.elites_next[(size_t)r * HD + e] = xs[r];
            }
        }
        if (wg == 0 && tid < m.K) m.elites_cost_next[tid] = key_cost(sel[tid]);
        __syncthreads();
        if (ra.dbg && tid == 0 && wg == 0) ra.dbg[6] = wall_clock64();
        if (!REC && ra.dbg && tid == 0 && wg == 0) ra.dbg[7] = wall_clock64();
        if (has_row && r_mine < sa.n) {
            const float lo = lo_reg, hi = hi_reg;
            for (int t = QS ? q : 0; t < H; t += QS ? 4 : 1) {
                const float v = __builtin_fmaf(trow[t * D], mrow[HD + t * D], mrow[t * D]);
                trow[t * D] = __builtin_amdgcn_fmed3f(v, lo, hi);
            }
        }
    }
    if (tid < 32) {
        float ov = obs_reg;
        asm volatile("" : "+v"(ov));
        obs_stage[tid] = tid < ra.o ? ov : 0.f;
    }
    if (ra.dbg && tid == 0 && wg == 0) ra.dbg[10] = wall_clock64();
    __syncthreads();
    if (sa.row0_mean && sa.first_index + base == 0) {
        for (int e = tid; e < HD; e += NTT) tile_rows[e] = ms[e];
        __syncthreads();
    }
    {
        const int total4 = (n_rows - base < TPB ? n_rows - base : TPB) * (HD / VW);
        const Vec* t4 = reinterpret_cast<const Vec*>(tile_rows);
        Vec* g4 = reinterpret_cast<Vec*>(sa.out + (size_t)base * HD);
        constexpr int CP0 = (NTT - 64 * RWV >= 128) ? 64 * RWV : 0;
        if (tid >= CP0)
            for (int e = tid - CP0; e < total4; e += NTT - CP0) g4[e] = t4[e];
    }
    if (ra.dbg && tid == 0 && wg == 0) ra.dbg[11] = wall_clock64();
    unsigned long long run_key = KEY_SENTINEL;
    if constexpr (T4) {
        if (wave < RWV) {
            tile.load_obs(obs_stage);
            const int rs = wave * 4 + (lane >> 4);
            const int row = base + rs;
            const float* rd = tile.read_ptr(tilebuf, rs, HD);
            const float* ar = tile.row_ptr(tilebuf, rs, HD);
            typename Tile::State st;
            tile.init(st);
#pragma unroll
            for (int t = 0; t < H; ++t) tile.step(st, rd + t * D, ar + t * D);
            const float cost = tile.cost(st);
            const bool live = row < n_rows;
            if ((lane & 15) == 0) {
                if (live) ra.costs[row] = cost;
                note_nonfinite(ra, cost, live);
                wg_keys[0][0][rs] = (live && row < ra.n_cand) ? make_key(cost, row)
                                    : TPB <= 16 ? KEY_SENTINEL : ((KEY_SENTINEL & 0xFFFFFFFF00000000ull) | (KEY_FILL_LO + (unsigned)rs));
            }
        }
        if (ra.dbg && tid == 0 && wg == 0) ra.dbg[13] = wall_clock64();
        if (ra.K > 0 && wg < n_wg) {
            __syncthreads();
            if (wave == 0 && TPB <= 16) {
                const unsigned long long key = wave_sort_first<16>(lane < TPB ? wg_keys[0][0][lane] : KEY_SENTINEL, lane);
                if (lane < ra.K) {
                    if (ra.part_k) {
                        ra.part_k[(size_t)lane * n_wg + wg] = key;
                    } else {
                        ra.part_c[(size_t)wg * ra.K + lane] = key_cost(key);
                        ra.part_i[(size_t)wg * ra.K + lane] = key_idx(key);
                    }
                }
            } else if (wave == 0) {
                constexpr int NK = TPB <= 16 ? 16 : 32, PARTS = 64 / NK, PER = NK / PARTS;
                static_assert(TPB <= 32 && PER % 2 == 0, "one wave counts for the slab");
                const unsigned long long* keys = &wg_keys[0][0][0];
                const int i = lane & (NK - 1), part = lane / NK;
                const unsigned long long mine = i < TPB ? keys[i] : KEY_SENTINEL;
                unsigned place = 0;
#pragma unroll
                for (int c = 0; c < PER; ++c) {
                    const int e = part * PER + c;
                    place += (e < TPB && keys[e < TPB ? e : 0] < mine) ? 1u : 0u;
                }
                if (NK == 16) place += (unsigned)__shfl_xor((int)place, 16, 64);
                place += (unsigned)__shfl_xor((int)place, 32, 64);
                if (part == 0 && i < TPB && place < (unsigned)ra.K) {
                    const bool filler = (mine >> 32) == (KEY_SENTINEL >> 32) && (unsigned)mine >= KEY_FILL_LO;
                    const unsigned long long key = filler ? KEY_SENTINEL : mine;
                    if (ra.part_k) {
                        ra.part_k[(size_t)place * n_wg + wg] = key;
                    } else {
                        ra.part_c[(size_t)wg * ra.K + place] = key_cost(key);
                        ra.part_i[(size_t)wg * ra.K + place] = key_idx(key);
                    }
                }
            }
        }
    } else {
        if (wave < RW) {
            tile.load_obs(obs_stage);
            run_key = rollout_slab<Tile, H, D, true>(tile, ra, rd0, base + wave * 16 + (lane & 15), n_rows, run_key, true, lane);
            if (ra.dbg && tid == 0 && wg == 0) ra.dbg[12] = wall_clock64();
        }
        if (ra.dbg && tid == 0 && wg == 0) ra.dbg[13] = wall_clock64();
        if (ra.K > 0 && wg < n_wg) wg_merge_emit<RW>(wg_keys, run_key, ra.K, lane, wave, ra, wg, n_wg);
    }
    if (ra.dbg && tid == 0 && wg == 0) ra.dbg[14] = wall_clock64();
}


template <int H, int D, int O, int KIND, int ROUNDS, int RW, int KREG, bool REC, int ARITH>
__global__ __launch_bounds__(sr_threads(D, RW) + (KREG > 0 ? 64 : 0)) void sample_rollout_kernel(FastIterArgs a) {
    sample_rollout_body<H, D, O, KIND, ROUNDS, RW, KREG, REC, ARITH>(a.s, a.r, a.m, a.p);
}

template <int H, int D, int O, int KIND, int ROUNDS, int RW, int KREG, int ARITH>
__global__ __launch_bounds__(sr_threads(D, RW) + (KREG > 0 ? 64 : 0)) void sample_rollout_batch_kernel(const FastIterArgs* __restrict__ args,
                                                                                                      BatchBases bases) {
    const FastIterArgs& a = args[blockIdx.y];
    FastSampleArgs s = from_device(a.s);
    const unsigned long long base = bases.v[blockIdx.y];
    add_base64(s.off_lo, s.off_hi, base);
    add_base64(s.off2_lo, s.off2_hi, base);
    const FastRolloutArgs r = from_device(a.r);
    const MergeSingleArgs m = from_device(a.m);
    sample_rollout_body<H, D, O, KIND, ROUNDS, RW, KREG, false, ARITH>(s, r, m, a.p);
}

}

constexpr int single_launch_max_rw(int h, int d) {
    int best = 0;
    for (int rw = 1; rw <= 8; rw *= 2)
        if (sr_threads(d, rw) + 64 <= 1024 && 16 * rw * h * d * 4 <= 120 * 1024) best = rw;
    return best;
}

static bool sample_rollout_shape(const BatchHint& bh, int h, int d, int O, int rounds, int n_rows, int n_tail, int* grid_out, int* rw_out,
                                 int* tail_out = nullptr) {
    const int max_rw = opt_i(OPT_FUSE_MAX_RW);
    int grid, rw, tail = 0;
    r16_shape(n_rows, &grid, &rw);
    const int mult = bh.mult;
    if (mult > 1) {
        int g_all, rw_all;
        r16_shape(n_rows * mult, &g_all, &rw_all);
        const int cap = opt_i(OPT_BATCH_MAX_RW);
        rw = std::min(std::max(rw, rw_all), std::min(cap > 0 ? cap : 8, single_launch_max_rw(h, d)));
        while (rw > 1 && rw > single_launch_max_rw(h, d)) rw /= 2;
        grid = (std::max(1, (n_rows + 15) / 16) + rw - 1) / rw;
        if (grid > FAST_MAX_LISTS) return false;
    } else
    if (n_tail > 0 && n_tail <= 64) {
        int g2, w2;
        r16_shape(n_rows - n_tail, &g2, &w2);
        if (w2 < rw && sr_threads(d, w2) + 64 <= 512 && g2 == FAST_MAX_LISTS && n_rows - n_tail == FAST_MAX_LISTS * 16 * w2) {
            rw = w2;
            tail = n_tail;
        }
    }
    if (rounds != 10 || rw > max_rw || n_rows <= 0 || !fast_rollout_supported(h, d, O, 1) || !fast_sample_supported(h, d))
        return false;
    if (rw > single_launch_max_rw(h, d)) return false;
    *grid_out = tail ? (n_rows + 16 * rw - 1) / (16 * rw) : std::min(grid, (n_rows + 16 * rw - 1) / (16 * rw));
    *rw_out = rw;
    if (tail_out) *tail_out = tail;
    return true;
}

int sample_rollout_lists(const BatchHint& bh, int h, int d, int O, int rounds, int n_rows, int n_tail, int* tail_out) {
    int grid, rw, tail = 0;
    if (!sample_rollout_shape(bh, h, d, O, rounds, n_rows, n_tail, &grid, &rw, &tail)) return 0;
    if (tail_out) *tail_out = tail;
    return tail ? FAST_MAX_LISTS : grid;
}

bool sample_rollout_merge_ok(const BatchHint& bh, int h, int d, int O, int rounds, int n_rows, int K) {
    const int on = opt_i(OPT_MERGE_PROLOGUE);
    int grid, rw;
    return on && K + 1 <= 12 && sample_rollout_shape(bh, h, d, O, rounds, n_rows, 0, &grid, &rw);
}

bool sample_rollout_pack_ok(const BatchHint& bh, int h, int d, int O, int rounds, int n_rows, int K) {
    const int on = opt_i(OPT_RIDING_PACK);
    int grid, rw;
    return on && sample_rollout_merge_ok(bh, h, d, O, rounds, n_rows, K) && sample_rollout_shape(bh, h, d, O, rounds, n_rows, 0, &grid, &rw) &&
           K * (h * d + 2) <= 16 * rw * h * d;
}

namespace {
template <int H, int D, int O, int KIND, int RW, int KREG, bool REC, int ARITH>
struct SrInst {
    static constexpr int THREADS = sr_threads(D, RW) + (KREG > 0 ? 64 : 0);
    static constexpr bool BATCHED = !REC;
    static void solo(int grid, hipStream_t st, const FastIterArgs& a) {
        hipLaunchKernelGGL((sample_rollout_kernel<H, D, O, KIND, 10, RW, KREG, REC, ARITH>), dim3(grid), dim3(THREADS), 0, st, a);
    }
    static void batch(int grid, int n, hipStream_t st, const FastIterArgs* args_dev, const BatchBases& bases) {
        hipLaunchKernelGGL((sample_rollout_batch_kernel<H, D, O, KIND, 10, RW, KREG, ARITH>), dim3(grid, n), dim3(THREADS), 0, st, args_dev, bases);
    }
};
template <int H, int D, int O, int RW, class F>
bool sample_rollout_pick(const LaunchKey& k, F& f) {
    if constexpr (RW > single_launch_max_rw(H, D)) {
        return false;
    } else {
        if (k.waves != RW) return false;
        auto with = [&](auto kind, auto arith) {
            constexpr int KK = decltype(kind)::value, AA = decltype(arith)::value;
            if (k.form == 2) f(SrInst<H, D, O, KK, RW, 12, true, AA>{});
            else if (k.form == 1) f(SrInst<H, D, O, KK, RW, 12, false, AA>{});
            else f(SrInst<H, D, O, KK, RW, 0, false, AA>{});
            return true;
        };
        using I0 = std::integral_constant<int, 0>;
        using I1 = std::integral_constant<int, 1>;
        if constexpr (O <= 20) {
            if (k.arith == 1) return k.kind == 1 ? with(I1{}, I1{}) : with(I0{}, I1{});
        }
        return k.kind == 1 ? with(I1{}, I0{}) : with(I0{}, I0{});
    }
}
template <class F>
bool sample_rollout_dispatch(const LaunchKey& k, F&& f) {
#define XR(HH, DD, OO)                                                                                      \
    if (k.h == HH && k.d == DD && k.O == OO)                                                                \
        return sample_rollout_pick<HH, DD, OO, 1>(k, f) || sample_rollout_pick<HH, DD, OO, 2>(k, f) ||      \
               sample_rollout_pick<HH, DD, OO, 4>(k, f) || sample_rollout_pick<HH, DD, OO, 8>(k, f);
    ICEM_FAST_SHAPES(XR)
#undef XR
    return false;
}
}

void launch_sample_rollout(const LaunchCtx& cx, const FastIterArgs& a, int h, int d, int O, int kind, bool merge_prologue) {
    LaunchKey k;
    if (!sample_rollout_shape(cx.hint, h, d, O, 10, a.r.n_rows, a.r.list_wgs > 0 ? a.s.n_shift : 0, &k.wgs[0], &k.waves)) return;
    k.family = LAUNCH_SAMPLE_ROLLOUT;
    k.h = h, k.d = d, k.O = O, k.kind = kind, k.arith = a.r.arith;
    k.form = !merge_prologue ? 0 : a.m.records ? 2 : 1;
    k.wgs[1] = (k.form == 2 && a.p.part_k) ? 1 : 0;
    submit(cx, k, k.form != 2, [&](void* dst, unsigned long long base) { batch_form(a, base, dst); },
           [&] { sample_rollout_dispatch(k, [&](auto inst) { inst.solo(k.wgs[0] + k.wgs[1], cx.st, a); }); });
}

void launch_sample_rollout_batch(const LaunchKey& k, const FastIterArgs* args_dev, const BatchBases& bases, int n, hipStream_t st) {
    sample_rollout_dispatch(k, [&](auto inst) {
        if constexpr (decltype(inst)::BATCHED) inst.batch(k.wgs[0], n, st, args_dev, bases);
    });
}

}
```

icem_amd/csrc/k_merge.hip:

```cpp
#include "fused_dev.h"
#include "refit.h"

namespace icem {

namespace {

template <int KREG, bool REC>
__device__ __forceinline__ void merge_single_body(const MergeSingleArgs& a, unsigned char* smem_raw) {
    __shared__ unsigned long long sel[64];
    __shared__ unsigned long long cand[64];
    __shared__ int slot[64];
    typedef float __attribute__((address_space(3))) * LdsF;
    const LdsF new_mean = (LdsF)smem_raw;
    const int tid = threadIdx.x;
    const int lane = tid & 63;
    const int hd = a.h * a.d;
    if (a.dbg && threadIdx.x == 0) a.dbg[0] = wall_clock64();
    constexpr int EPL = 4;
    const bool pre = hd <= MERGE_WG * EPL;
    float om[EPL], os[EPL], blo[EPL], bhi[EPL];
#pragma unroll
    for (int i = 0; i < EPL; ++i) {
        const int e = tid + i * MERGE_WG;
        om[i] = (pre && e < hd) ? a.mean[e] : 0.f;
        os[i] = (pre && e < hd) ? a.std[e] : 0.f;
    }
    auto request_bounds = [&]() {
#pragma unroll
        for (int i = 0; i < EPL; ++i) {
            const int e = tid + i * MERGE_WG;
            blo[i] = (pre && a.last && e < hd) ? a.low[e % a.d] : 0.f;
            bhi[i] = (pre && a.last && e < hd) ? a.high[e % a.d] : 0.f;
        }
    };
    if (REC || tid >= 64) request_bounds();
    if constexpr (REC) {
        merge_select_records_wg(a, tid < 64, lane, tid, MERGE_WG, sel, slot);
        if (a.dbg && threadIdx.x == 0) a.dbg[4] = wall_clock64();
    } else {
        if (tid < 64) merge_select_shallow<3>(a, lane, cand, sel);
        if (a.dbg && threadIdx.x == 0) a.dbg[4] = wall_clock64();
        if (tid < 64) request_bounds();
        __syncthreads();
    }
    const float* rows[KREG];
    merge_rows<KREG, REC>(a, sel, slot, rows);
    float best0 = 0.f;
    auto finish_one = [&](int e, float old_mean, float old_std) {
        float xs[KREG];
#pragma unroll
        for (int r = 0; r < KREG; ++r) xs[r] = rows[r][e];
#pragma unroll
        for (int r = 0; r < KREG; ++r) asm volatile("" : "+v"(xs[r]));
        float nm, ns;
        refit_element_regs<float, KREG>(a.K, a.alpha, old_mean, old_std, xs, nm, ns);
#pragma unroll
        for (int r = 0; r < KREG; ++r)
            if (r < a.K) a.elites_next[(size_t)r * hd + e] = xs[r];
        if (!a.last) {
            a.mean_out[e] = nm;
            a.std_out[e] = ns;
        } else {
            new_mean[e] = nm;
        }
        if (e == tid) best0 = xs[0];
    };
    if (pre) {
#pragma unroll
        for (int i = 0; i < EPL; ++i) {
            const int e = tid + i * MERGE_WG;
            if (e < hd) finish_one(e, om[i], os[i]);
        }
    } else {
        for (int e = tid; e < hd; e += MERGE_WG) finish_one(e, a.mean[e], a.std[e]);
    }
    if (a.dbg && threadIdx.x == 0) a.dbg[5] = wall_clock64();
    if (tid < a.K) a.elites_cost_next[tid] = key_cost(sel[tid]);
    if (a.last) {
        __syncthreads();
        if (pre) {
#pragma unroll
            for (int i = 0; i < EPL; ++i) {
                const int e = tid + i * MERGE_WG;
                if (e < hd) {
                    a.mean_out[e] = (e + a.d < hd) ? new_mean[e + a.d] : new_mean[e];
                    a.std_out[e] = (bhi[i] - blo[i]) / 2.f * a.init_std;
                }
            }
        } else {
            for (int e = tid; e < hd; e += MERGE_WG) {
                const int j = e % a.d;
                a.mean_out[e] = (e + a.d < hd) ? new_mean[e + a.d] : new_mean[e];
                a.std_out[e] = (a.high[j] - a.low[j]) / 2.f * a.init_std;
            }
        }
        if (tid < a.d) a.executed[tid] = best0;
        if (tid == 0) a.best_cost[0] = key_cost(sel[0]);
    }
    if (a.dbg && threadIdx.x == 0) a.dbg[6] = wall_clock64();
}

template <int KREG, bool REC>
__global__ __launch_bounds__(MERGE_WG) void merge_single_kernel(MergeSingleArgs a) {
    extern __shared__ __attribute__((aligned(16))) unsigned char smem_raw[];
    merge_single_body<KREG, REC>(a, smem_raw);
}

template <int H, int KREG>
__global__ __launch_bounds__(MERGE_WG) void merge_noise_kernel(MergeSingleArgs a, FastSampleArgs z1, FastSampleArgs z2, int wgs1) {
    extern __shared__ __attribute__((aligned(16))) unsigned char smem_raw[];
    if (blockIdx.x == 0) {
        merge_single_body<KREG, false>(a, smem_raw);
        return;
    }
    const bool second = (int)blockIdx.x > wgs1;
    const FastSampleArgs& z = second ? z2 : z1;
    float* tile = reinterpret_cast<float*>(smem_raw);
    const int d = z.d, hd = H * d, tpw = MERGE_WG / d, tid = threadIdx.x;
    const int n_base = ((int)blockIdx.x - 1 - (second ? wgs1 : 0)) * tpw;
    const int n_here = cmin(tpw, z.n - n_base);
    if (tid < n_here * d) {
        const int nl = tid / d;
        const int j = tid - nl * d;
        float* trow = tile + nl * hd + j;
        sample_row<H, 10>(z.W, (unsigned)(z.first_index + n_base + nl), (unsigned)j, z.off_lo, z.off_hi, z.seed_lo, z.seed_hi,
                          [&](int t, float y) { trow[t * d] = y; }, z.white != 0);
    }
    __syncthreads();
    float* gdst = z.out + (size_t)n_base * hd;
    const int total = n_here * hd;
    if ((hd & 3) == 0) {
        const float4* t4 = reinterpret_cast<const float4*>(tile);
        float4* g4 = reinterpret_cast<float4*>(gdst);
        for (int e = tid; e < total / 4; e += MERGE_WG) g4[e] = t4[e];
    } else {
        for (int e = tid; e < total; e += MERGE_WG) gdst[e] = tile[e];
    }
}

template <int H, int KREG>
__global__ __launch_bounds__(MERGE_WG) void merge_noise_batch_kernel(const MergeNoiseBatchArgs* __restrict__ args, BatchBases bases, int wgs1) {
    extern __shared__ __attribute__((aligned(16))) unsigned char smem_raw[];
    const MergeNoiseBatchArgs& g = args[blockIdx.y];
    if (blockIdx.x == 0) {
        const MergeSingleArgs a = from_device(g.a);
        merge_single_body<KREG, false>(a, smem_raw);
        return;
    }
    const bool second = (int)blockIdx.x > wgs1;
    const FastSampleArgs z = from_device(second ? g.z2 : g.z1);
    float* tile = reinterpret_cast<float*>(smem_raw);
    const int d = z.d, hd = H * d, tpw = MERGE_WG / d, tid = threadIdx.x;
    const int n_base = ((int)blockIdx.x - 1 - (second ? wgs1 : 0)) * tpw;
    const int n_here = cmin(tpw, z.n - n_base);
    if (n_here <= 0) return;
    uint32_t off_lo = z.off_lo, off_hi = z.off_hi;
    add_base64(off_lo, off_hi, bases.v[blockIdx.y]);
    if (tid < n_here * d) {
        const int nl = tid / d;
        const int j = tid - nl * d;
        float* trow = tile + nl * hd + j;
        sample_row<H, 10>(z.W, (unsigned)(z.first_index + n_base + nl), (unsigned)j, off_lo, off_hi, z.seed_lo, z.seed_hi,
                          [&](int t, float y) { trow[t * d] = y; }, z.white != 0);
    }
    __syncthreads();
    float* gdst = z.out + (size_t)n_base * hd;
    const int total = n_here * hd;
    if ((hd & 3) == 0) {
        const float4* t4 = reinterpret_cast<const float4*>(tile);
        float4* g4 = reinterpret_cast<float4*>(gdst);
        for (int e = tid; e < total / 4; e += MERGE_WG) g4[e] = t4[e];
    } else {
        for (int e = tid; e < total; e += MERGE_WG) gdst[e] = tile[e];
    }
}

constexpr size_t PACK_STAGE_MAX = 48 * 1024;

template <int KREG>
__global__ __launch_bounds__(MERGE_WG) void pack_records_kernel(MergeSingleArgs a, int n_loc, int shard_lo, float* records, XchgPush px) {
    __shared__ unsigned long long sel[64];
    __shared__ unsigned long long cand[64];
    extern __shared__ __attribute__((aligned(16))) float stage[];
    const int tid = threadIdx.x;
    if (tid < 64) merge_select<KREG>(a, tid, cand, sel);
    __syncthreads();
    pack_records_body<KREG>(a, n_loc, shard_lo, records, px, stage, sel, tid, MERGE_WG);
}

template <int KREG>
__global__ __launch_bounds__(MERGE_WG) void pack_merge_kernel(MergeSingleArgs pk, int n_loc, int shard_lo, float* records, XchgPush px,
                                                               MergeSingleArgs m) {
    __shared__ unsigned long long sel[64];
    __shared__ unsigned long long cand[64];
    extern __shared__ __attribute__((aligned(16))) unsigned char smem_raw[];
    const int tid = threadIdx.x;
    if (tid < 64) merge_select<KREG>(pk, tid, cand, sel);
    __syncthreads();
    pack_records_body<KREG>(pk, n_loc, shard_lo, records, px, reinterpret_cast<float*>(smem_raw), sel, tid, MERGE_WG);
    __syncthreads();
    merge_single_body<KREG, true>(m, smem_raw);
}

__global__ __launch_bounds__(1024) void topk_small_kernel(const float* costs, int n, int K, float* out_c, int* out_i) {
    __shared__ unsigned long long wg_keys[2][16][32];
    const int lane = threadIdx.x & 63, wave = threadIdx.x >> 6;
    unsigned long long run = KEY_SENTINEL;
    bool first = true;
    for (int base = wave * 64; base < n; base += 1024) {
        const int i = base + lane;
        unsigned long long key = wave_sort64(i < n ? make_key(costs[i], i) : KEY_SENTINEL, lane);
        if (!first) {
            const unsigned long long prev = __shfl(run, lane - 32, 64);
            key = (lane >= 32 && lane < 32 + K) ? prev : (lane < K ? key : KEY_SENTINEL);
            key = wave_sort64(key, lane);
        }
        run = key;
        first = false;
    }
    FastRolloutArgs fr{};
    fr.part_c = out_c;
    fr.part_i = out_i;
    wg_merge_emit<16>(wg_keys, run, K, lane, wave, fr, 0, 1);
}

template <bool FINISH>
__device__ __forceinline__ void update_small_body(const UpdateSmallArgs& a, const UpdateFinishArgs* f) {
    __shared__ unsigned long long wg_keys[2][16][32];
    __shared__ unsigned long long sel[32];
    __shared__ float shifted[FINISH ? UPDATE_FINISH_MAX_HD : 1];
    const int tid = threadIdx.x, lane = tid & 63, wave = tid >> 6;
    const int n_all = a.n + a.n_keep;
    unsigned long long run = KEY_SENTINEL;
    bool first = true;
    for (int base = wave * 64; base < n_all; base += 1024) {
        const int i = base + lane;
        unsigned long long key = KEY_SENTINEL;
        if (i < n_all) key = make_key(i < a.n ? a.costs[i] : a.keep_costs[i - a.n], i);
        key = wave_sort64(key, lane);
        if (!first) {
            const unsigned long long prev = __shfl(run, lane - 32, 64);
            key = (lane >= 32 && lane < 32 + a.K) ? prev : (lane < a.K ? key : KEY_SENTINEL);
            key = wave_sort64(key, lane);
        }
        run = key;
        first = false;
    }
    FastRolloutArgs fr{};
    fr.part_k = sel;
    wg_merge_emit<16>(wg_keys, run, a.K, lane, wave, fr, 0, 1);
    __syncthreads();
    if (tid < a.K) {
        a.elite_costs_out[tid] = key_cost(sel[tid]);
        a.idx_out[tid] = key_idx(sel[tid]);
    }
    auto row = [&](int r) -> const float* {
        int i = key_idx(sel[r]);
        if (i < 0 || i == INT_MAX) i = key_idx(sel[0]);
        return i < a.n ? a.pool + (size_t)i * a.hd : a.keep_actions + (size_t)(i - a.n) * a.hd;
    };
    for (int e = tid; e < a.hd; e += 1024) {
        for (int r = 0; r < a.K; ++r) a.elites_out[(size_t)r * a.hd + e] = row(r)[e];
        float nm, ns;
        refit_element<float>(a.K, a.alpha, a.mean[e], a.std[e], [&](int r) { return row(r)[e]; }, nm, ns);
        if (FINISH) {
            shifted[e] = nm;
        } else {
            a.mean[e] = nm;
            a.std[e] = ns;
        }
    }
    if (FINISH) {
        __syncthreads();
        const int d = f->d;
        for (int e = tid; e < a.hd; e += 1024) {
            const int j = e % d;
            a.mean[e] = (e + d < a.hd) ? shifted[e + d] : shifted[e];
            a.std[e] = (f->high[j] - f->low[j]) / 2.f * f->init_std;
        }
        if (tid < d) {
            const float x = row(0)[tid];
            f->executed[tid] = x;
            if (f->result) f->result[tid] = x;
        }
// ... 115 lines not shown
```

icem_amd/csrc/options.h:

```cpp
#pragma once

namespace icem {

#define ICEM_OPTIONS(X)                                                                                                   \
    X(DISABLE_FAST, "disable_fast", 0.0)              \
    X(FUSE_MAX_RW, "fuse_max_rw", 8.0)                \
    X(MERGE_PROLOGUE, "merge_prologue", 1.0)                                      \
    X(RIDING_PACK, "riding_pack", 1.0)                             \
    X(PUBLISHED_MERGE, "published_merge", 1.0)             \
    X(PACK_MERGE, "pack_merge", 1.0)                  \
    X(NOISE_AHEAD, "noise_ahead", 1.0)                             \
    X(NOISE_AHEAD_MIN_ROWS, "noise_ahead_min_rows", 0.0)                                                                \
    X(NOISE_AHEAD_SHARDED, "noise_ahead_sharded", 1.0)                                                                     \
    X(AHEAD_STAMPS, "ahead_stamps", 0.0)                                                                                   \
    X(AHEAD_TAIL_FRAC, "ahead_tail_frac", 0.4)                                                                             \
    X(AHEAD_NEXT1_FRAC, "ahead_next1_frac", 0.3)                                                                           \
    X(AHEAD_NOISE_LDS_KB, "ahead_noise_lds_kb", -1.0)                                                                      \
    X(PREDRAW, "predraw", 1.0)                              \
    X(GK_SAMPLE, "gk_sample", 1.0)                          \
    X(GK_ROLLOUT_THREAD, "gk_rollout_thread", 0.0)                   \
    X(GK_SELECT, "gk_select", 1.0)                                    \
    X(HN_PAIR, "hn_pair", 1.0)                                                               \
    X(HN_SPLIT, "hn_split", 1.0)                                                                                           \
    X(RSSM_SPLIT, "rssm_split", 1.0)                                                                                       \
    X(RSSM_SPLIT_MAX_N, "rssm_split_max_n", 65536.0)                                                                       \
    X(RSSM_SPLIT_TT, "rssm_split_tt", 0.0)                                                                                 \
    X(BATCH_AHEAD, "batch_ahead", 1.0)                \
    X(BATCH_AHEAD_MIN_ROWS, "batch_ahead_min_rows", 49152.0)    \
    X(BATCH_MAX_RW, "batch_max_rw", 0.0)              \
    X(LEARNED_STEP, "learned_step", 1.0)              \
    X(XCHG_LOOPBACK, "xchg_loopback", 0.0)            \
    X(XCHG_MAX_POLLS, "xchg_max_polls", 0.0)
enum Opt {
#define X(id, name, def) OPT_##id,
    ICEM_OPTIONS(X)
#undef X
    OPT_COUNT
};
double opt(Opt k);
inline int opt_i(Opt k) { return (int)opt(k); }

}
```

icem_amd/csrc/plan.hip:

```cpp
#include "host_common.h"
#include "cost_terms_dev.h"

using namespace icem;

__global__ void publish_result_kernel(const float* executed, const float* best_cost, const unsigned* nonfinite, int d, float* host_out,
                                      unsigned* flag, unsigned seq) {
    const int j = threadIdx.x;
    if (j < d) host_out[j] = executed[j];
    if (j == d) host_out[d] = best_cost[0];
    if (j == d + 1) reinterpret_cast<unsigned*>(host_out)[d + 1] = nonfinite[0];
    __threadfence_system();
    __syncthreads();
    if (j == 0) __hip_atomic_store(flag, seq, __ATOMIC_RELEASE, __HIP_MEMORY_SCOPE_SYSTEM);
}

namespace icem {

template <class T>
static T zeroed_args() {
    T t;
    std::memset((void*)&t, 0, sizeof(T));
    return t;
}

// ... 498 lines not shown
    return ICEM_OK;
}

template <typename T>
int plan_iter_local_t(icem_handle* h, const icem_plan_buffers* b, int mpc_step, int it, const LaunchCtx& cx) {
    hipStream_t st = cx.st;
    const icem_config& c = h->cfg;
    const int hd = h->hd, K = c.num_elites;
    const int n_global = h->pop[it];
    const Shard sh = shard_of(h, it);
    const int lo = sh.lo, n_loc = sh.n_loc;
    const uint64_t base = call_base(h, mpc_step);
    const bool last = it == c.opt_iters - 1;
    T* actions = (T*)b->actions;
    const int n_extra = shift_rows(h, mpc_step, it);
    const T* shift_src = nullptr;
    bool shift_in_sampler = false;
    if (n_extra > 0) {
        shift_src = (const T*)b->elites + (size_t)elite_parity(h, mpc_step, 0) * K * hd;
        shift_in_sampler = std::is_same<T, float>::value && b->z_r == nullptr && b->z_r_shift == nullptr &&
                           fast_rollout_ok(h, K) && fast_sample_ok(h) &&
                           n_extra * c.act_dim <= 256;
        if (!shift_in_sampler) {
            T* dst = actions + (size_t)n_loc * hd;
            int rc = gk_shift_elites(h, n_extra, shift_src, dst, cx);
            if (rc) return rc;
            rc = gk_sample(h, n_extra, 0, b->mean, b->std, b->low, b->high, b->z_r_shift, b->z_i_shift,
                           base + (uint64_t)c.opt_iters, c.horizon - 1, 0, dst, cx);
            if (rc) return rc;
        }
    }
    const int n_cand = n_loc + (c.rank == 0 ? n_extra : 0);
    const int row0 = (last && c.use_mean_actions) ? 1 : 0;
    T* rec = (T*)b->records + (size_t)c.rank * K * (hd + 2);
    h->local.lists = 0;
    h->local.sel_cand = 0;
    if constexpr (std::is_same<T, float>::value) {
        if (fast_rollout_ok(h, K)) {
            const bool ext_z = b->z_r != nullptr;
            const uint64_t off = base + (uint64_t)it;
            int rc = ensure_fast_model(h);
            if (rc) return rc;
            int lists = 0;
            float* pc;
            int* pi;
            const int n_rows = n_loc + n_extra;
            int tail_rows = 0;
            const int one = (!ext_z && fast_sample_ok(h) && (n_extra == 0 || shift_in_sampler))
                                ? one_launch_lists(h, cx.hint, n_rows, shift_in_sampler ? n_extra : 0, &tail_rows) : 0;
            h->local.tail_rows = one > 0 ? tail_rows : 0;
            split_partial_ws<float>(b->workspace, one > 0 ? one : rollout_lists(c.horizon, c.act_dim, h->Of, n_rows), K, &pc, &pi);
            bool prologue = false, ride = false;
            if (h->ride.merge_pending) {
                prologue = !ext_z && n_extra == 0 && prologue_possible(h, cx.hint, n_rows);
                ride = prologue && h->ride.pack_pending && next_launch_takes_pack(h, cx.hint, n_rows);
                if (h->ride.pack_pending && !ride) {
                    rc = launch_pending_pack(h, cx);
                    if (rc) return rc;
                }
                if (!prologue) {
                    rc = launch_pending_merge(h, cx);
                    if (rc) return rc;
                }
                h->ride.merge_pending = false;
            } else if (h->ride.pack_pending) {
                rc = launch_pending_pack(h, cx);
                if (rc) return rc;
            }
            h->ride.pack_pending = false;
            if (one > 0) {
                FastIterArgs fa = zeroed_args<FastIterArgs>();
                fa.m.keep_base = -1;
                if (prologue) fa.m = h->ride.merge;
                if (ride) fa.p = h->ride.pack;
                fa.s = fast_sample_args(h, n_loc, lo, b->mean, b->std, b->low, b->high, off, row0, actions,
                                        shift_in_sampler ? n_extra : 0, shift_src, base + (uint64_t)c.opt_iters);
                if (it == 0 && c.world == 1 && h->ahead.pre_valid) {
                    if (h->ahead.pre_episode == h->episode && h->ahead.pre_step == mpc_step && h->ahead.pre_stream == st) fa.s.raw_src = (const float*)h->ahead.pre_raw;
                    h->ahead.pre_valid = false;
                }
                fa.r = fast_rollout_args(h, n_rows, n_cand, K, b->obs0, actions, b->costs, pc, pi);
                fa.r.part_k = (unsigned long long*)b->workspace;
                fa.r.list_wgs = tail_rows > 0 ? one : 0;
                {
                    ProfScope prof(h, ICEM_K_SAMPLE_ROLLOUT, (long long)n_rows * c.horizon, st);
                    launch_sample_rollout(cx, fa, c.horizon, c.act_dim, h->Of, h->model_kind, prologue);
                }
                ICEM_HIP_TRY(hipGetLastError());
                lists = one;
            }
            if (one == 0) {
                if (prologue) {
                    FastSampleMergeArgs sm = zeroed_args<FastSampleMergeArgs>();
                    sm.s = fast_sample_args(h, n_loc, lo, b->mean, b->std, b->low, b->high, off, row0, actions, 0, nullptr, 0);
                    sm.m = h->ride.merge;
                    if (ride) {
                        sm.p = h->ride.pack;
                        const int pub_on = opt_i(OPT_PUBLISHED_MERGE);
                        if (pub_on && sm.m.records) {
                            rc = ensure_pub(h, st);
                            if (rc) return rc;
                            set_pub(h, sm.p);
                        }
                    }
                    {
                        ProfScope prof(h, ICEM_K_SAMPLE, (long long)n_loc * c.horizon, st);
                        launch_sample_folded_merge(cx, sm);
                    }
                    ICEM_HIP_TRY(hipGetLastError());
                    rc = ICEM_OK;
                } else if (ext_z) {
                    rc = gk_sample(h, n_loc, lo, b->mean, b->std, b->low, b->high, b->z_r, b->z_i, off, 0, row0, actions, cx);
                } else if (fast_sample_ok(h)) {
                    rc = launch_fast_sample(h, n_loc, lo, b->mean, b->std, b->low, b->high, off, row0, actions, cx,
                                            shift_in_sampler ? n_extra : 0, shift_src, base + (uint64_t)c.opt_iters);
                } else {
                    rc = gk_sample(h, n_loc, lo, b->mean, b->std, b->low, b->high, nullptr, nullptr, off, 0, row0, actions, cx);
                }
                if (rc) return rc;
                int tail2 = 0;
                rc = launch_fast_rollout(h, n_rows, n_cand, K, b->obs0, actions, b->costs, pc, pi, cx, &lists,
                                         (unsigned long long*)b->workspace, (c.world == 1 && it == 0) ? n_extra : 0, &tail2);
                if (rc) return rc;
                h->local.tail_rows = tail2;
            }
            h->local.lists = lists;
            if (c.world > 1) {
                const MergeSingleArgs pk = local_pack_args(h, it, lists, n_rows, b->workspace, (const float*)actions, n_loc,
                                                           (one > 0 && c.rank == 0) ? tail_rows : 0, b->costs);
                XchgPush px;
                const bool fold_push = xchg_connected(h) && pack_can_push(K, c.horizon, c.act_dim);
                if (fold_push) {
                    rc = xchg_begin(h, &px, &h->xw_last);
                    if (rc) return rc;
                }
                const int fuse_last = opt_i(OPT_PACK_MERGE);
                const bool rides_next = !last && it + 1 < c.opt_iters;
                if (fold_push && xchg_concurrent_peers(h) && h->deferral && (rides_next || (last && fuse_last)) && lists > 0 && records_fit_prologue(h)) {
                    const int n_next = rides_next ? shard_of(h, it + 1).n_loc : 0;
                    if (!rides_next || (prologue_possible(h, cx.hint, n_next) && next_launch_takes_pack(h, cx.hint, n_next))) {
                        h->ride.pack = make_pack(pk, sh, (float*)rec, px);
                        h->ride.pack_pending = true;
                        return ICEM_OK;
                    }
                }
                {
                    ProfScope prof(h, ICEM_K_LOCAL_PACK, lists * K, st);
                    launch_pack_records(pk, n_loc, lo, (float*)rec, st, px);
                }
                ICEM_HIP_TRY(hipGetLastError());
                if (xchg_connected(h) && !fold_push) return xchg_push(h, rec, st, &h->xw_last);
            }
            ICEM_HIP_TRY(hipGetLastError());
            return ICEM_OK;
        }
    }
    int rc = gk_sample(h, n_loc, lo, b->mean, b->std, b->low, b->high, b->z_r, b->z_i, base + (uint64_t)it, 0, row0,
                       actions, cx);
    if (rc) return rc;
    rc = gk_rollout(h, n_loc + n_extra, b->obs0, actions, b->costs, nullptr, cx);
    if (rc) return rc;
    h->local.sel_cand = 0;
    if (c.world == 1 && gk_select_ok(h, n_cand, h->n_reuse, K)) {
        h->local.sel_cand = n_cand;
        h->local.sel_loc = n_loc;
        return ICEM_OK;
    }
// ... 523 lines not shown
    if (rc) return rc;
    rc = ensure_pp_stats(h);
    if (rc) return rc;
    const bool last = it == h->cfg.opt_iters - 1;
    const bool fold = !last && h->local.lists > 0 && records_fit_prologue(h) && prologue_possible(h, cx.hint, shard_of(h, it + 1).n_loc);
    icem_plan_buffers bb = *b;
    bb.mean = h->cur_mean;
    bb.std = h->cur_std;
    const MergeRoute route = merge_route(h, b, it, fold);
    rc = plan_iter_merge_t<float>(h, &bb, mpc_step, it, cx, route);
    if (rc) return rc;
    if (fold && h->ride.merge_pending) {
        h->cur_mean = route.mean_out;
        h->cur_std = route.std_out;
    }
    if (last) h->cur_mean = h->cur_std = nullptr;
    return ICEM_OK;
}

static void disarm(icem_handle* h) {
    h->ride.clear();
    h->local.clear();
    h->ahead.tail_pending = h->ahead.next_valid = h->ahead.pre_valid = false;
    h->ahead.next1_rows = 0;
}
static int disarm_on_error(icem_handle* h, int rc) {
    if (rc != ICEM_OK) disarm(h);
    return rc;
}

static int plan_step_sharded_body(icem_handle* h, const icem_plan_buffers* b, int32_t mpc_step, void* stream) {
    if (h->cfg.world < 2) return icem_plan_step(h, b, mpc_step, stream);
    if (!xchg_connected(h) && !rccl_connected(h))
        return fail(ICEM_E_STATE, "neither the in-library exchange (icem_exchange_create / _connect) nor an RCCL communicator "
                                  "(icem_rccl_connect / _adopt) is connected");
    if (b && b->z_r != nullptr) return fail(ICEM_E_INVALID, "external noise goes through icem_plan_iter_local / _merge");
    if (xchg_status_peek(h) & 1u)
        return fail(ICEM_E_STATE, "in-library exchange: a wait for a peer's elite records timed out in an earlier MPC step "
                                  "(icem_exchange_status reads and clears the word); the plans since then are not valid");
    if (b && check_plan(h, b, mpc_step, 0, (hipStream_t)stream) == ICEM_OK && !h->ride.merge_pending && !h->ride.pack_pending && ahead_eligible(h, b, BatchHint(), true))
        return plan_step_sharded_ahead(h, b, mpc_step, LaunchCtx{(hipStream_t)stream});
    const bool was = h->deferral;
    h->deferral = true;
    int rc = ICEM_OK;
    const bool by_rccl = !xchg_connected(h);
    for (int it = 0; it < h->cfg.opt_iters && rc == ICEM_OK; ++it) {
        rc = icem_plan_iter_local(h, b, mpc_step, it, stream);
        if (rc == ICEM_OK && by_rccl) rc = rccl_allgather_records(h, b->records, (hipStream_t)stream);
        if (rc == ICEM_OK) rc = icem_plan_iter_merge(h, b, mpc_step, it, stream);
    }
    h->deferral = was;
    return rc;
}

int icem_plan_step_sharded(icem_handle* h, const icem_plan_buffers* b, int32_t mpc_step, void* stream) {
    if (check_handle(h)) return ICEM_E_INVALID;
    return disarm_on_error(h, plan_step_sharded_body(h, b, mpc_step, stream));
}

static int plan_step_body(icem_handle* h, const icem_plan_buffers* b, int32_t mpc_step, const LaunchCtx& cx) {
    if (h->cfg.world != 1) return fail(ICEM_E_INVALID, "icem_plan_step is the world == 1 path; use iter_local/iter_merge");
    int rc = check_plan(h, b, mpc_step, 0, cx.st);
    if (rc) return rc;
    const icem_config& c = h->cfg;
    const int iters = c.opt_iters;
    if (ahead_eligible(h, b, cx.hint)) return plan_step_ahead(h, b, mpc_step, cx);
    const bool pingpong = c.dtype == ICEM_F32 && b->z_r == nullptr && h->use_fast && iters > 1;
    if (pingpong && !h->actions_alt) ICEM_HIP_TRY(hipMalloc(&h->actions_alt, icem_plan_buffer_bytes(h, ICEM_BUF_ACTIONS)));
    if (pingpong && !h->ws_alt) ICEM_HIP_TRY(hipMalloc(&h->ws_alt, icem_plan_buffer_bytes(h, ICEM_BUF_WORKSPACE)));
    if (pingpong) {
        rc = ensure_pp_stats(h);
        if (rc) return rc;
    }
    float* cur_mean = (float*)b->mean;
    float* cur_std = (float*)b->std;
    for (int it = 0; it < iters; ++it) {
        icem_plan_buffers bb = *b;
        if (pingpong) {
            if ((iters - 1 - it) & 1) bb.actions = h->actions_alt;
            if (it & 1) bb.workspace = h->ws_alt;
            bb.mean = cur_mean;
            bb.std = cur_std;
        }
        rc = ICEM_DISPATCH(h, plan_iter_local_t<float>(h, &bb, mpc_step, it, cx), plan_iter_local_t<double>(h, &bb, mpc_step, it, cx));
        if (rc) return rc;
        const bool last = it == iters - 1;
        if (last) predraw_next_step(h, b, mpc_step, cx);
        bool fold = false;
        if (pingpong && !last && h->local.lists > 0) fold = prologue_possible(h, cx.hint, h->pop[it + 1]);
        const MergeRoute route = merge_route(h, b, it, fold);
        rc = ICEM_DISPATCH(h, plan_iter_merge_t<float>(h, &bb, mpc_step, it, cx, route), plan_iter_merge_t<double>(h, &bb, mpc_step, it, cx, route));
        if (rc) return rc;
        if (last && h->ahead.tail_pending) {
            h->ahead.tail_pending = false;
            h->ahead.pre_valid = false;
        }
        if (fold && h->ride.merge_pending) {
            cur_mean = route.mean_out;
            cur_std = route.std_out;
        }
    }
    return ICEM_OK;
}

int icem_plan_step(icem_handle* h, const icem_plan_buffers* b, int32_t mpc_step, void* stream) {
    if (check_handle(h)) return ICEM_E_INVALID;
    return disarm_on_error(h, plan_step_body(h, b, mpc_step, LaunchCtx{(hipStream_t)stream}));
}


static const char* batch_ineligible(icem_handle* h, const icem_plan_buffers* b, int32_t mpc_step, const BatchHint& bh) {
    const icem_config& c = h->cfg;
    const int K = c.num_elites;
    if (c.world != 1) return "world must be 1";
    if (c.dtype != ICEM_F32 || !h->use_fast) return "dtype f32 on the throughput kernels only";
    if (b->z_r || b->z_i || b->z_r_shift || b->z_i_shift) return "external noise is not batched";
    if (h->profiling || h->dbg) return "per-kernel profiling / debug stamps are per handle: switch them off";
    const bool gemm = gemm_rollout(h) && !h->hn_tile;
    if (!fast_rollout_ok(h, K) || !fast_sample_ok(h) || K + 1 > 12 || c.rng_rounds != 10)
        return (h->hn_tile || gemm) ? "the merge cannot ride in the sampler's prologue (num_elites <= 11, the default generator)" : "shape outside the single-launch kernels";
    if (h->ride.merge_pending || h->ride.pack_pending) return "a deferred merge is pending: finish the MPC step first";
    if (c.opt_iters < 1) return "opt_iters";
    if (gemm && !sample_batch_compiled(c.horizon)) return "the batched samplers of a GEMM-kernel shape are compiled for horizon 30 only";
    if (h->hn_tile || gemm) {
        if (h->pop.empty() || h->pop[0] > 8192) return "populations above 8192 rows per iteration are not batched: they fill the chip by themselves";
        if (shift_rows(h, mpc_step, 0, false) * c.act_dim > 256) return "too many shifted elites for the sampling launch";
        if (c.opt_iters > 1 && !sample_folded_merge_ok(c.horizon, c.act_dim, c.rng_rounds, K))
            return "an iteration cannot carry the previous merge in its prologue";
        return nullptr;
    }
    if (ahead_eligible(h, b, BatchHint()))
        return "populations that take the noise-ahead launches alone (> 8192 rows per iteration) are not batched: they fill the chip by themselves";
    if (ahead_eligible(h, b, bh)) return nullptr;
    for (int it = 0; it < c.opt_iters; ++it) {
        const int n_extra = shift_rows(h, mpc_step, it, false);
        if (n_extra * c.act_dim > 256) return "too many shifted elites for the sampling launch";
        if (one_launch_lists(h, bh, h->pop[it] + n_extra, n_extra) <= 0) return "an iteration's population has no single-launch kernel";
        if (it > 0 && !prologue_possible(h, bh, h->pop[it])) return "an iteration cannot carry the previous merge in its prologue";
    }
    return nullptr;
}

static int run_recorded_batch(icem_handle* const* handles, int n, const icem_plan_buffers* buffers, int32_t mpc_step, hipStream_t st,
                              const BatchHint& hint, const std::string& who, size_t spare, long long* launches_out) {
    struct DisarmGuard {
        icem_handle* const* handles;
        int n;
        bool armed = true;
        ~DisarmGuard() {
            for (int i = 0; armed && i < n; ++i) disarm(handles[i]);
        }
    } disarm_all{handles, n};
    BatchBases bases{};
    std::vector<LaunchRecorder> recs(n);
    int rc = ICEM_OK;
    bool unsupported = false;
    for (int i = 0; i < n && rc == ICEM_OK; ++i) {
        recs[i].base = bases.v[i] = call_base(handles[i], mpc_step);
        recs[i].who = who.c_str();
        recs[i].launches.reserve(3 * handles[i]->cfg.opt_iters + 2);
        rc = plan_step_body(handles[i], &buffers[i], mpc_step, LaunchCtx{st, hint, &recs[i]});
        unsupported = unsupported || recs[i].unsupported;
    }
    if (rc == ICEM_OK && unsupported) rc = fail(ICEM_E_UNSUPPORTED, who + "a launch without a batched form was reached");
    const std::vector<LaunchDesc>& first = recs[0].launches;
    const size_t L = first.size();
    for (int i = 0; i < n && rc == ICEM_OK; ++i) {
        if (recs[i].launches.size() != L || L == 0) rc = fail(ICEM_E_STATE, who + "the problems' steps took different launches");
        for (size_t l = 0; l < L && rc == ICEM_OK; ++l)
// ... 200 lines not shown
```

icem_amd/planner.py:

```python
from __future__ import annotations

import ctypes as C
import os
from dataclasses import dataclass
from typing import Callable, Optional, Sequence, Tuple

import numpy as np
import torch

from . import _lib as L
from .distributed import exchange_records, shard_range


@dataclass
class IcemConfig:
    horizon: int
    act_dim: int
    num_traj: int
    elites_size: int = 10
    opt_iters: int = 3
    cost_mode: str = "sum"
    use_mean_actions: bool = True
    keep_previous_elites: bool = True
    shift_elites: bool = True
# ... 198 lines not shown
        n = costs.shape[0]
        k = self.K if k is None else k
        nbytes = self.lib.icem_topk_workspace_bytes(self._h, n, k)
        if self._topk_ws is None or self._topk_ws.numel() < nbytes:
            self._topk_ws = torch.empty((max(nbytes, 1),), dtype=torch.uint8, device=self.device)
        out_c = torch.empty((k,), dtype=self.dt, device=self.device)
        out_i = torch.empty((k,), dtype=torch.int32, device=self.device)
        L.check(self.lib.icem_topk_sorted(self._h, n, _ptr(costs), k, _ptr(out_c), _ptr(out_i), _ptr(self._topk_ws),
                                          self._stream()))
        return out_c, out_i

    def gather_refit(self, actions: torch.Tensor, idx: torch.Tensor, mean: torch.Tensor, std: torch.Tensor):
        assert mean.dtype == self.dt and std.dtype == self.dt and mean.is_contiguous() and std.is_contiguous()
        actions = self._t(actions)
        idx = idx.to(device=self.device, dtype=torch.int32).contiguous()
        k = idx.shape[0]
        elites = torch.empty((k, self.h, self.d), dtype=self.dt, device=self.device)
        L.check(self.lib.icem_gather_refit(self._h, _ptr(actions), _ptr(idx), k, _ptr(mean), _ptr(std), _ptr(elites),
                                           self._stream()))
        return elites

    def can_update_in_one_launch(self, n_all: int, k: int) -> bool:
        return bool(self.lib.icem_update_distribution_ok(self._h, int(n_all), int(k)))

    def update_distribution(self, costs: torch.Tensor, pool: torch.Tensor, k: int, mean: torch.Tensor, std: torch.Tensor,
                            keep_costs: Optional[torch.Tensor] = None, keep_actions: Optional[torch.Tensor] = None):
        assert mean.dtype == self.dt and std.dtype == self.dt and mean.is_contiguous() and std.is_contiguous()
        n = costs.shape[0]
        costs, pool = self._t(costs, (n,)), self._t(pool, (n, self.h, self.d))
        n_keep = 0 if keep_costs is None else keep_costs.shape[0]
        if n_keep:
            keep_costs, keep_actions = self._t(keep_costs, (n_keep,)), self._t(keep_actions, (n_keep, self.h, self.d))
        elites = torch.empty((k, self.h, self.d), dtype=self.dt, device=self.device)
        ec = torch.empty(k, dtype=self.dt, device=self.device)
        idx = torch.empty(k, dtype=torch.int32, device=self.device)
        L.check(self.lib.icem_update_distribution(self._h, n, _ptr(costs), _ptr(pool), n_keep,
                                                  _ptr(keep_costs) if n_keep else None, _ptr(keep_actions) if n_keep else None,
                                                  k, _ptr(mean), _ptr(std), _ptr(elites), _ptr(ec), _ptr(idx), self._stream()))
        return ec, idx, elites

    def sample_truncnorm(self, n: int, mean, std, lower, upper, u=None, offset: int = 0, first_index: int = 0,
                         out: Optional[torch.Tensor] = None) -> torch.Tensor:
        mean, std = self._t(mean, (self.h, self.d)), self._t(std, (self.h, self.d))
        lower, upper = self._t(lower, (self.h, self.d)), self._t(upper, (self.h, self.d))
        if u is not None:
            u = self._t(u, (n, self.h, self.d))
        if out is None:
            out = torch.empty((n, self.h, self.d), dtype=self.dt, device=self.device)
        L.check(self.lib.icem_sample_truncnorm(self._h, n, first_index, _ptr(mean), _ptr(std), _ptr(lower), _ptr(upper),
                                               _ptr(u), offset, _ptr(out), self._stream()))
        return out

    def cem_bounds(self, mean: torch.Tensor, std: torch.Tensor, like_levine: bool):
        assert mean.dtype == self.dt and std.dtype == self.dt and mean.is_contiguous() and std.is_contiguous()
        lower = torch.empty((self.h, self.d), dtype=self.dt, device=self.device)
        upper = torch.empty_like(lower)
        L.check(self.lib.icem_cem_bounds(self._h, int(like_levine), _ptr(mean), _ptr(std), _ptr(self.low), _ptr(self.high),
                                         _ptr(lower), _ptr(upper), self._stream()))
        return lower, upper

    def shift(self, mean: torch.Tensor, std: torch.Tensor):
        L.check(self.lib.icem_shift(self._h, _ptr(mean), _ptr(std), _ptr(self.low), _ptr(self.high), self._stream()))

    def reset_distribution(self, mean: torch.Tensor, std: torch.Tensor):
        L.check(self.lib.icem_reset_distribution(self._h, _ptr(mean), _ptr(std), _ptr(self.low), _ptr(self.high),
                                                 self._stream()))

    def set_tile_arith(self, mode="auto"):
        m = {"auto": -1, "f32": 0, "f16x2": 1}.get(mode, mode)
        L.check(self.lib.icem_set_tile_arith(self._h, int(m)))
        return self.tile_arith

    @property
    def tile_arith(self):
        return int(self.lib.icem_tile_arith(self._h))

    @property
    def tile_growth(self) -> float:
        return float(self.lib.icem_tile_growth(self._h))

    def nonfinite_costs(self) -> int:
        n = C.c_int64()
        L.check(self.lib.icem_nonfinite_costs(self._h, C.byref(n), self._stream()))
        return int(n.value)

    F64_ARITH = {"chain": 0, "mfma": 1}

    def set_f64_arith(self, mode="chain"):
        m = self.F64_ARITH.get(mode, mode)
        L.check(self.lib.icem_set_f64_arith(self._h, int(m)))
        return self.f64_arith

    @property
    def f64_arith(self):
        return {0: "chain", 1: "mfma"}[int(self.lib.icem_f64_arith(self._h))]

    WIDE_ARITH = {"auto": -1, "f16x2": 0, "fp16x2": 0, "f32": 1, "bf16x3": 2}

    def set_wide_arith(self, mode="auto"):
        m = self.WIDE_ARITH.get(mode, mode)
        L.check(self.lib.icem_set_wide_arith(self._h, int(m)))
        return self.wide_arith

    @property
    def wide_arith(self):
        return {0: "f16x2", 1: "f32", 2: "bf16x3"}[int(self.lib.icem_wide_arith(self._h))]

    @property
    def wide_imbalance_log2(self):
        return int(self.lib.icem_wide_imbalance_log2(self._h))

    def set_wide_exact(self, on=True):
        L.check(self.lib.icem_set_wide_exact(self._h, int(on)))

    def profile_enable(self, on: bool = True):
        L.check(self.lib.icem_profile_enable(self._h, int(on)))

    def profile_read(self):
        n = len(L.KERNEL_NAMES)
        ms, cnt, units = (C.c_double * n)(), (C.c_int64 * n)(), (C.c_int64 * n)()
        L.check(self.lib.icem_profile_read(self._h, ms, cnt, units))
        return {L.KERNEL_NAMES[i]: (ms[i], cnt[i], units[i]) for i in range(n) if cnt[i]}

    def profile_overhead(self, reps: int = 200, spin_us: float = 15.0) -> Tuple[float, float]:
        pair, kern = C.c_double(), C.c_double()
        L.check(self.lib.icem_profile_overhead(self._stream(), reps, spin_us, C.byref(pair), C.byref(kern)))
        return pair.value, kern.value

    def get_action_host(self, obs) -> Tuple[np.ndarray, float]:
        self._ensure_buffers()
        self._cb.z_r = self._cb.z_i = self._cb.z_r_shift = self._cb.z_i_shift = None
        ob = np.ascontiguousarray(obs, dtype=np.float64)
        if ob.shape != (self.obs_dim,):
            raise ValueError(f"expected an observation of shape ({self.obs_dim},)")
        act = np.empty(self.d, dtype=np.float64)
        best = C.c_double()
        rc = self.lib.icem_get_action(self._h, C.byref(self._cb), self.mpc_step, ob.ctypes.data_as(C.POINTER(C.c_double)),
                                      act.ctypes.data_as(C.POINTER(C.c_double)), C.byref(best), self._stream())
        if rc in (0, L.ICEM_E_RANGE):
            self.mpc_step += 1
        L.check(rc)
        return act, best.value

    def plan_step_resident(self):
        self._cb.z_r = self._cb.z_i = self._cb.z_r_shift = self._cb.z_i_shift = None
        st = self._stream()
        if self.cfg.world == 1:
            L.check(self.lib.icem_plan_step(self._h, C.byref(self._cb), self.mpc_step, st))
        elif getattr(self, "_exchange", False) or getattr(self, "_rccl", False):
            L.check(self.lib.icem_plan_step_sharded(self._h, C.byref(self._cb), self.mpc_step, st))
        else:
            self._set_deferral(True)
            gather = self._resident_gather()
            local, merge, cb, h, step = self.lib.icem_plan_iter_local, self.lib.icem_plan_iter_merge, C.byref(self._cb), self._h, self.mpc_step
            for it in range(self.cfg.opt_iters):
                L.check(local(h, cb, step, it, st))
                gather()
                L.check(merge(h, cb, step, it, st))
        self.mpc_step += 1

    @staticmethod
    def plan_step_batch(planners: Sequence["IcemPlanner"], observations=None):
        return IcemPlanner._step_batch("icem_plan_step_batch", planners, observations)

    @staticmethod
    def _step_batch(entry: str, planners, observations):
# ... 327 lines not shown
```

include/icem_hip.h:

```cpp
#ifndef ICEM_HIP_H
#define ICEM_HIP_H

#include <stddef.h>
#include <stdint.h>

#ifdef __cplusplus
extern "C" {
#endif

#define ICEM_ABI_VERSION 6

enum { ICEM_F32 = 0, ICEM_F64 = 1 };
enum { ICEM_COST_SUM = 0, ICEM_COST_BEST = 1, ICEM_COST_FINAL = 2 };
enum { ICEM_MODEL_LINEAR = 0, ICEM_MODEL_TANH = 1 };

enum {
    ICEM_OK = 0,
    ICEM_E_INVALID = -1,
    ICEM_E_UNSUPPORTED = -2,
    ICEM_E_HIP = -3,
    ICEM_E_NO_DEVICE = -4,
    ICEM_E_STATE = -5,
    ICEM_E_RANGE = -6
};
// ... 129 lines not shown

typedef struct icem_plan_buffers {
    void* mean;
    void* std;
    void* low;
    void* high;
    void* obs0;
    void* actions;
    void* costs;
    void* elites;
    void* records;
    void* workspace;
    void* executed;
    void* best_cost;
    const void* z_r;
    const void* z_i;
    const void* z_r_shift;
    const void* z_i_shift;
} icem_plan_buffers;

enum {
    ICEM_BUF_MEAN = 0, ICEM_BUF_STD, ICEM_BUF_LOW, ICEM_BUF_HIGH, ICEM_BUF_OBS0, ICEM_BUF_ACTIONS,
    ICEM_BUF_COSTS, ICEM_BUF_ELITES, ICEM_BUF_RECORDS, ICEM_BUF_WORKSPACE, ICEM_BUF_EXECUTED,
    ICEM_BUF_BEST_COST, ICEM_BUF_COUNT
};
size_t icem_plan_buffer_bytes(const icem_handle* h, int32_t which);

int icem_plan_iter_local(icem_handle* h, const icem_plan_buffers* b, int32_t mpc_step, int32_t it,
                         void* stream);
int icem_plan_iter_merge(icem_handle* h, const icem_plan_buffers* b, int32_t mpc_step, int32_t it,
                         void* stream);
int icem_set_merge_deferral(icem_handle* h, int32_t on);

#define ICEM_IPC_HANDLE_BYTES 64
int icem_exchange_create(icem_handle* h, void* ipc_handle_out_host);
int icem_exchange_connect(icem_handle* h, const void* handles_host, void* const* local_blocks);
void* icem_exchange_block(icem_handle* h);
int icem_exchange_disable(icem_handle* h);
int icem_exchange_status(icem_handle* h, int32_t* status_host, int32_t* finegrained_host);
int icem_exchange_probe(icem_handle* h, int32_t rounds, void* stream, double* us_out);
#define ICEM_RCCL_ID_BYTES 128
int icem_rccl_load(const char* path_or_null);
const char* icem_rccl_library(void);
int icem_rccl_unique_id(void* id_out_host);
int icem_rccl_connect(icem_handle* h, const void* id_host);
int icem_rccl_adopt(icem_handle* h, void* nccl_comm);
int icem_rccl_disconnect(icem_handle* h);
int icem_allgather_elites(icem_handle* h, void* records, void* stream);

int icem_plan_step_sharded(icem_handle* h, const icem_plan_buffers* b, int32_t mpc_step, void* stream);

int icem_plan_step(icem_handle* h, const icem_plan_buffers* b, int32_t mpc_step, void* stream);

int icem_plan_step_batch(icem_handle* const* handles, int32_t n, const icem_plan_buffers* buffers, int32_t mpc_step, void* stream);
int64_t icem_batch_uploads(const icem_handle* h);

int icem_plan_step_batch_f64(icem_handle* const* handles, int32_t n, const icem_plan_buffers* buffers, int32_t mpc_step, void* stream);
int64_t icem_batch_f64_launches(const icem_handle* h);

#define ICEM_RSSM_OBS_DIM 230
int icem_plan_step_learned_ok(const icem_handle* h);
int icem_plan_step_learned(icem_handle* h, const icem_plan_buffers* b, const void* params, int32_t mpc_step, void* stream);
int icem_plan_step_learned_batch(icem_handle* const* handles, int32_t n, const icem_plan_buffers* buffers, const void* params,
                                 const int32_t* mpc_steps_host, void* results, void* stream);
int64_t icem_learned_step_launches(const icem_handle* h);

enum { ICEM_WIDE_AUTO = -1, ICEM_WIDE_F16X2 = 0, ICEM_WIDE_F32 = 1, ICEM_WIDE_BF16X3 = 2 };
int icem_set_wide_arith(icem_handle* h, int32_t mode);
int icem_wide_arith(const icem_handle* h);
int icem_wide_imbalance_log2(const icem_handle* h);
int icem_wide_model_imbalance_log2(int32_t obs_dim, int32_t act_dim, const double* A_host, const double* B_host);
int icem_set_wide_exact(icem_handle* h, int32_t on);

enum { ICEM_TILE_AUTO = -1, ICEM_TILE_F32 = 0, ICEM_TILE_F16X2 = 1 };
int icem_set_tile_arith(icem_handle* h, int32_t mode);
int icem_tile_arith(const icem_handle* h);
double icem_tile_growth(const icem_handle* h);

enum { ICEM_F64_CHAIN = 0, ICEM_F64_MFMA = 1 };
int icem_set_f64_arith(icem_handle* h, int32_t mode);
int icem_f64_arith(const icem_handle* h);

int icem_nonfinite_costs(icem_handle* h, int64_t* count_out, void* stream);

int icem_set_option(const char* name, double value);
int icem_get_option(const char* name, double* value_out);
int icem_reset_options(void);
const char* icem_option_name(int32_t index);

enum {
    ICEM_K_SAMPLE = 0, ICEM_K_ROLLOUT, ICEM_K_TOPK_PARTIAL, ICEM_K_LOCAL_PACK, ICEM_K_MERGE_REFIT,
    ICEM_K_SAMPLE_ROLLOUT, ICEM_K_COUNT
};
int icem_profile_enable(icem_handle* h, int32_t on);
int icem_debug_stamps(icem_handle* h, void* dev_ptr);
int icem_profile_read(icem_handle* h, double* total_ms, int64_t* launches, int64_t* units);
int icem_profile_overhead(void* stream, int32_t reps, double spin_us, double* pair_us, double* kernel_us);

size_t icem_record_bytes(const icem_handle* h);

size_t icem_rssm_param_elems(void);
int icem_rssm_trim(void);
int icem_rssm_rollout_cost(int32_t n, int32_t horizon, int32_t cost_mode, const void* params, const void* obs0,
                           const void* actions, void* costs, void* stream);
int icem_rssm_rollout_cost_batch(int32_t n_problems, const int32_t* rows_host, int32_t horizon, int32_t cost_mode,
                                 const void* params, const void* obs0, const void* actions, void* costs, void* stream);

int icem_get_action(icem_handle* h, const icem_plan_buffers* b, int32_t mpc_step, const double* obs_host,
                    double* action_host, double* best_cost_host, void* stream);

#ifdef __cplusplus
}
#endif
#endif
```

Before: 7.663 billion.

## Fold final-iteration merge into sample-rollout kernel via last-block ticket

On the last CEM iteration, the sample-rollout kernel now takes an atomic ticket per workgroup, and the last workgroup to finish performs the final elite merge/refit and writes mean, std, executed action and best cost. This removes the separate merge kernel launch and its dependency gap. Extra workgroups in the same grid also draw the next step's predrawn noise rows. Partial top-k lists and outputs are written with agent-scope atomic stores and read back with atomic loads so the last block sees them, which may slow those stores and adds a serial tail on one block.

```diff
diff --git a/icem_amd/_lib.py b/icem_amd/_lib.py
--- a/icem_amd/_lib.py
+++ b/icem_amd/_lib.py
@@ -145,6 +145,7 @@
     ("icem_learned_step_launches", C.c_int64, [_H]),
     ("icem_tile_growth", C.c_double, [_H]),
     ("icem_nonfinite_costs", C.c_int, [_H, C.POINTER(C.c_int64), _VP]),
+    ("icem_last_merge_ticket", C.c_int, [_H, C.POINTER(C.c_int64), _VP]),
     ("icem_set_option", C.c_int, [C.c_char_p, C.c_double]),
     ("icem_get_option", C.c_int, [C.c_char_p, C.POINTER(C.c_double)]),
     ("icem_reset_options", C.c_int, []),
@@ -156,6 +157,9 @@
 RCCL_ID_BYTES = 128
 RSSM_OBS_DIM = 230
 ABI_VERSION = 6
+
+
+SINCE_PARENT = {"icem_last_merge_ticket"}
 
 
 def lib_path() -> str:
@@ -172,6 +176,8 @@
                           f" or python -m icem_amd.build)")
     lib = C.CDLL(path)
     for name, res, args in SYMBOLS:
+        if name in SINCE_PARENT and not hasattr(lib, name):
+            continue
         fn = getattr(lib, name)
         fn.restype = res
         fn.argtypes = args
diff --git a/icem_amd/csrc/abi.hip b/icem_amd/csrc/abi.hip
--- a/icem_amd/csrc/abi.hip
+++ b/icem_amd/csrc/abi.hip
@@ -234,9 +234,12 @@
     if (!rc && (hipMalloc((void**)&h->nonfinite_dev, 2 * sizeof(unsigned)) != hipSuccess ||
                 hipMemset(h->nonfinite_dev, 0, 2 * sizeof(unsigned)) != hipSuccess))
         rc = fail(ICEM_E_HIP, "hipMalloc of the handle's status word failed");
+    if (!rc && (hipMalloc((void**)&h->ticket_dev, 128) != hipSuccess || hipMemset(h->ticket_dev, 0, 128) != hipSuccess))
+        rc = fail(ICEM_E_HIP, "hipMalloc of the handle's ticket counter failed");
     if (rc) {
         if (h->W_dev) (void)hipFree(h->W_dev);
         if (h->nonfinite_dev) (void)hipFree(h->nonfinite_dev);
+        if (h->ticket_dev) (void)hipFree(h->ticket_dev);
         delete h;
         return rc;
     }
@@ -251,6 +254,7 @@
     ahead_destroy(h);
     if (h->W_dev) (void)hipFree(h->W_dev);
     if (h->nonfinite_dev) (void)hipFree(h->nonfinite_dev);
+    if (h->ticket_dev) (void)hipFree(h->ticket_dev);
     if (h->actions_alt) (void)hipFree(h->actions_alt);
     if (h->host_stage) (void)hipHostFree(h->host_stage);
     if (h->ws_alt) (void)hipFree(h->ws_alt);
@@ -418,6 +422,20 @@
     return ICEM_OK;
 }
 
+int icem_last_merge_ticket(icem_handle* h, int64_t* count_out, void* stream) {
+    if (check_handle(h)) return ICEM_E_INVALID;
+    if (!count_out) return fail(ICEM_E_INVALID, "null output");
+    hipStream_t st = (hipStream_t)stream;
+    hipStreamCaptureStatus cap = hipStreamCaptureStatusNone;
+    if (hipStreamIsCapturing(st, &cap) == hipSuccess && cap != hipStreamCaptureStatusNone)
+        return fail(ICEM_E_STATE, "icem_last_merge_ticket synchronises: not on a capturing stream");
+    unsigned v = 0;
+    ICEM_HIP_TRY(hipMemcpyAsync(&v, h->ticket_dev, sizeof(v), hipMemcpyDeviceToHost, st));
+    ICEM_HIP_TRY(hipStreamSynchronize(st));
+    *count_out = (int64_t)v;
+    return ICEM_OK;
+}
+
 int icem_set_model(icem_handle* h, int32_t kind, int32_t obs_dim, const double* A_host, const double* B_host) {
     if (!h || !A_host || !B_host) return fail(ICEM_E_INVALID, "null argument");
     if (kind != ICEM_MODEL_LINEAR && kind != ICEM_MODEL_TANH) return fail(ICEM_E_INVALID, "model kind");
diff --git a/icem_amd/csrc/fused_dev.h b/icem_amd/csrc/fused_dev.h
--- a/icem_amd/csrc/fused_dev.h
+++ b/icem_amd/csrc/fused_dev.h
@@ -992,6 +992,17 @@
     __device__ __forceinline__ float cost(const State& st) const { return use_min ? st.acc_b : st.acc_s; }
 };
 
+template <bool WT, typename T>
+__device__ __forceinline__ void st_wt(T* p, T v) {
+    if constexpr (WT) __hip_atomic_store(p, v, __ATOMIC_RELAXED, __HIP_MEMORY_SCOPE_AGENT);
+    else *p = v;
+}
+template <bool AG, typename T>
+__device__ __forceinline__ T ld_ag(const T* p) {
+    if constexpr (AG) return __hip_atomic_load(p, __ATOMIC_RELAXED, __HIP_MEMORY_SCOPE_AGENT);
+    else return *p;
+}
+
 template <bool LANE_MASK = true>
 __device__ __forceinline__ unsigned long long topk_push16(unsigned long long run_key, unsigned long long key, bool first,
                                                           int K, int lane) {
@@ -1003,14 +1014,14 @@
 }
 
 constexpr unsigned KEY_FILL_LO = 0x7FFFFE00u;
-template <int WAVES>
+template <int WAVES, bool WT = false>
 __device__ __forceinline__ void wg_merge_emit(unsigned long long (*wg_keys)[WAVES][32], unsigned long long run_key, int K,
                                               int lane, int wave, const FastRolloutArgs& a, int wg = blockIdx.x,
                                               int n_wg = gridDim.x) {
     static_assert(WAVES * 32 <= 512, "filler keys: one per slot");
     auto emit = [&](unsigned long long key, int place) {
         if (a.part_k) {
-            a.part_k[(size_t)place * n_wg + wg] = key;
+            st_wt<WT>(a.part_k + ((size_t)place * n_wg + wg), key);
         } else {
             a.part_c[(size_t)wg * K + place] = key_cost(key);
             a.part_i[(size_t)wg * K + place] = key_idx(key);
@@ -1121,10 +1132,11 @@
 
 __device__ __forceinline__ int keep_index0(const MergeSingleArgs& a) { return a.keep_base >= 0 ? a.keep_base : a.n_global; }
 
+template <bool AG = false>
 __device__ __forceinline__ float merge_keep_cost(const MergeSingleArgs& a, int lane) {
     const bool has = a.elites_cost_cur != nullptr;
     const float* src = has ? a.elites_cost_cur : reinterpret_cast<const float*>(a.part_k);
-    const float v = src[(has && lane < a.n_keep) ? lane : 0];
+    const float v = ld_ag<AG>(src + ((has && lane < a.n_keep) ? lane : 0));
     return has ? v : 0.f;
 }
 
@@ -1211,15 +1223,16 @@
     }
 }
 
+template <bool AG = false>
 __device__ __forceinline__ void merge_select_stream(const MergeSingleArgs& a, int lane, unsigned long long* cand,
                                                     unsigned long long* sel) {
     const int K = a.K, nl = a.n_lists;
     auto key_at = [&](int l, int i) -> unsigned long long {
         const int list = lane + l * 64;
-        const unsigned long long v = a.part_k[(size_t)(i < K ? i : 0) * nl + (list < nl ? list : 0)];
+        const unsigned long long v = ld_ag<AG>(a.part_k + ((size_t)(i < K ? i : 0) * nl + (list < nl ? list : 0)));
         return (list < nl && i < K) ? v : KEY_SENTINEL;
     };
-    const unsigned long long kept = lane < a.n_keep ? make_key(a.elites_cost_cur[lane], keep_index0(a) + lane) : KEY_SENTINEL;
+    const unsigned long long kept = lane < a.n_keep ? make_key(ld_ag<AG>(a.elites_cost_cur + lane), keep_index0(a) + lane) : KEY_SENTINEL;
     unsigned long long mine = kept;
 #pragma unroll
     for (int l = 0; l < LPL; ++l) {
@@ -1276,17 +1289,17 @@
     }
 }
 
-template <int DEPTH>
+template <int DEPTH, bool AG = false>
 __device__ __forceinline__ void merge_select_shallow(const MergeSingleArgs& a, int lane, unsigned long long* cand,
                                                      unsigned long long* sel) {
     const int K = a.K, nl = a.n_lists;
-    const float keep_cost = merge_keep_cost(a, lane);
+    const float keep_cost = merge_keep_cost<AG>(a, lane);
     unsigned long long k[LPL][DEPTH];
 #pragma unroll
     for (int l = 0; l < LPL; ++l) {
         const int list = lane + l * 64;
 #pragma unroll
-        for (int i = 0; i < DEPTH; ++i) k[l][i] = a.part_k[(size_t)(i < K ? i : 0) * nl + (list < nl ? list : 0)];
+        for (int i = 0; i < DEPTH; ++i) k[l][i] = ld_ag<AG>(a.part_k + ((size_t)(i < K ? i : 0) * nl + (list < nl ? list : 0)));
     }
 #pragma unroll
     for (int l = 0; l < LPL; ++l) {
@@ -1325,7 +1338,7 @@
 #pragma unroll 1
         for (int i = DEPTH; i < K; ++i) {
             const int list = lane + l * 64;
-            const unsigned long long v = list < nl ? a.part_k[(size_t)i * nl + list] : KEY_SENTINEL;
+            const unsigned long long v = list < nl ? ld_ag<AG>(a.part_k + ((size_t)i * nl + list)) : KEY_SENTINEL;
             if (!offer(v)) break;
         }
     }
@@ -1336,7 +1349,7 @@
         key = wave_sort_n(key, lane, n_cand);
         if (lane < K) sel[lane] = key;
     } else {
-        merge_select_stream(a, lane, cand, sel);
+        merge_select_stream<AG>(a, lane, cand, sel);
     }
 }
 
diff --git a/icem_amd/csrc/host_common.h b/icem_amd/csrc/host_common.h
--- a/icem_amd/csrc/host_common.h
+++ b/icem_amd/csrc/host_common.h
@@ -94,7 +94,10 @@
         icem::MergeSingleArgs merge;
         bool pack_pending = false;
         icem::PackPrev pack;
-        void clear() { merge_pending = pack_pending = false; }
+        bool last_armed = false, last_done = false;
+        float* last_mean_out = nullptr;
+        float* last_std_out = nullptr;
+        void clear() { merge_pending = pack_pending = last_armed = last_done = false; }
     } ride;
     bool deferral = false;
     float* cur_mean = nullptr;
@@ -114,6 +117,7 @@
     int tile_ratio_log2 = 0;
     unsigned* nonfinite_dev = nullptr;
     unsigned nonfinite_seen = 0;
+    unsigned* ticket_dev = nullptr;
     void* Mw_dev = nullptr;
     void* Mws_dev = nullptr;
     void* Mwh_dev = nullptr;
diff --git a/icem_amd/csrc/icem_fused.h b/icem_amd/csrc/icem_fused.h
--- a/icem_amd/csrc/icem_fused.h
+++ b/icem_amd/csrc/icem_fused.h
@@ -266,6 +266,20 @@
     MergeSingleArgs m;
     PackPrev p;
 };
+struct LastMergeArgs {
+    MergeSingleArgs fin;
+    FastSampleArgs z1, z2;
+    unsigned* ticket;
+    int n_tickets;
+    int noise_form;
+    int wgs1, wgs2;
+};
+struct FastLastArgs {
+    FastIterArgs it;
+    LastMergeArgs l;
+};
+bool sample_rollout_last_ok(const BatchHint& bh, int h, int d, int O, int kind, int arith, int rounds, int n_rows, int K, bool merge_prologue);
+void launch_sample_rollout_last(const LaunchCtx& cx, FastLastArgs& a, int h, int d, int O, int kind, bool merge_prologue);
 }
 #include "generic_args.h"
 namespace icem {
diff --git a/icem_amd/csrc/k_iter_small.hip b/icem_amd/csrc/k_iter_small.hip
--- a/icem_amd/csrc/k_iter_small.hip
+++ b/icem_amd/csrc/k_iter_small.hip
@@ -1,4 +1,5 @@
 #include "fused_dev.h"
+#include "merge_body.h"
 
 namespace icem {
 
@@ -7,10 +8,11 @@
 constexpr bool sr_quad(int d, int rw) { return rw <= 2 && ((4 * 16 * rw * d + 63) / 64) * 64 + 64 <= 1024; }
 constexpr int sr_threads(int d, int rw) { return (((sr_quad(d, rw) ? 4 : 1) * 16 * rw * d + 63) / 64) * 64; }
 
-template <int H, int D, int O, int KIND, int ROUNDS, int RW, int KREG, bool REC, int ARITH>
+template <int H, int D, int O, int KIND, int ROUNDS, int RW, int KREG, bool REC, int ARITH, bool LAST = false>
 __device__ __forceinline__ void sample_rollout_body(const FastSampleArgs& sa, const FastRolloutArgs& ra, const MergeSingleArgs& am,
-                                                    const PackPrev& ap) {
+                                                    const PackPrev& ap, const LastMergeArgs* lp = nullptr) {
     constexpr bool PM = KREG > 0;
+    static_assert(!LAST || !REC, "the folded last merge is the lists form's");
     constexpr bool QS = sr_quad(D, RW);
     constexpr bool T4 = QS && O <= 20 && sr_threads(D, RW) >= 256 * RW && ARITH == 0;
     using T16 = typename TileSel<H, D, O, KIND, ARITH>::type;
@@ -30,13 +32,40 @@
     __shared__ float obs_stage[32];
     constexpr int WROWS = H / 2 + 1;
     __shared__ __attribute__((aligned(16))) float Wl[QS ? NT / 64 : 1][QS ? WROWS * WQ_STRIDE : 4];
-    __shared__ unsigned long long sel[PM ? 64 : 1];
-    __shared__ unsigned long long cand[PM ? 64 : 1];
-    __shared__ int slot[PM ? 64 : 1];
+    __shared__ unsigned long long sel[PM || LAST ? 64 : 1];
+    __shared__ unsigned long long cand[PM || LAST ? 64 : 1];
+    __shared__ int slot[PM || LAST ? 64 : 1];
+    __shared__ unsigned my_ticket;
     float* tile_rows = tilebuf + T16::SLACK;
     const int tid = threadIdx.x;
     const int lane = tid & 63;
     const int wave = tid >> 6;
+    auto draw_rows = [&](const FastSampleArgs& z, int r0, int r1) {
+        for (int c0 = r0; c0 < r1; c0 += TPB) {
+            const int n_here = r1 - c0 < TPB ? r1 - c0 : TPB;
+            if (tid < n_here * D) {
+                const int nl = tid / D, j = tid - nl * D;
+                float* trow = tile_rows + nl * HD + j;
+                sample_row<H, ROUNDS>(z.W, (unsigned)(z.first_index + c0 + nl), (unsigned)j, z.off_lo, z.off_hi, z.seed_lo, z.seed_hi,
+                                      [&](int t, float y) { trow[t * D] = y; }, z.white != 0);
+            }
+            __syncthreads();
+            const Vec* t4 = reinterpret_cast<const Vec*>(tile_rows);
+            Vec* g4 = reinterpret_cast<Vec*>(z.out + (size_t)c0 * HD);
+            for (int e = tid; e < n_here * (HD / VW); e += NTT) g4[e] = t4[e];
+            __syncthreads();
+        }
+    };
+    if constexpr (LAST) {
+        const int nb = (int)blockIdx.x - lp->n_tickets;
+        if (nb >= 0) {
+            const bool second = nb >= lp->wgs1;
+            const FastSampleArgs& z = second ? lp->z2 : lp->z1;
+            const int r0 = (nb - (second ? lp->wgs1 : 0)) * TPB;
+            draw_rows(z, r0, r0 + TPB < z.n ? r0 + TPB : z.n);
+            return;
+        }
+    }
     const int n_rows = ra.n_rows;
     const bool has_pack = PM && REC && ap.part_k != nullptr;
     if constexpr (PM && REC) {
@@ -69,7 +98,7 @@
         }
     }
     const int wg = blockIdx.x - (has_pack ? 1 : 0);
-    const int n_wg = ra.list_wgs > 0 ? ra.list_wgs : (int)gridDim.x - (has_pack ? 1 : 0);
+    const int n_wg = LAST ? lp->n_tickets : ra.list_wgs > 0 ? ra.list_wgs : (int)gridDim.x - (has_pack ? 1 : 0);
     const int base = wg * TPB;
     if (base >= n_rows) return;
     if (ra.dbg && tid == 0 && wg == 0) ra.dbg[8] = wall_clock64();
@@ -240,14 +269,14 @@
             ms[e] = nm;
             ms[HD + e] = ns;
             if (wg == 0) {
-                m.mean_out[e] = nm;
-                m.std_out[e] = ns;
+                st_wt<LAST>(m.mean_out + e, nm);
+                st_wt<LAST>(m.std_out + e, ns);
 #pragma unroll
                 for (int r = 0; r < KREG; ++r)
-                    if (r < m.K) m.elites_next[(size_t)r * HD + e] = xs[r];
-            }
-        }
-        if (wg == 0 && tid < m.K) m.elites_cost_next[tid] = key_cost(sel[tid]);
+                    if (r < m.K) st_wt<LAST>(m.elites_next + ((size_t)r * HD + e), xs[r]);
+            }
+        }
+        if (wg == 0 && tid < m.K) st_wt<LAST>(m.elites_cost_next + tid, key_cost(sel[tid]));
         __syncthreads();
         if (ra.dbg && tid == 0 && wg == 0) ra.dbg[6] = wall_clock64();
         if (!REC && ra.dbg && tid == 0 && wg == 0) ra.dbg[7] = wall_clock64();
@@ -275,6 +304,12 @@
         const Vec* t4 = reinterpret_cast<const Vec*>(tile_rows);
         Vec* g4 = reinterpret_cast<Vec*>(sa.out + (size_t)base * HD);
         constexpr int CP0 = (NTT - 64 * RWV >= 128) ? 64 * RWV : 0;
+        if constexpr (LAST) {
+            const unsigned long long* t8 = reinterpret_cast<const unsigned long long*>(tile_rows);
+            unsigned long long* g8 = reinterpret_cast<unsigned long long*>(sa.out + (size_t)base * HD);
+            if (tid >= CP0)
+                for (int e = tid - CP0; e < total4 * (VW / 2); e += NTT - CP0) st_wt<true>(g8 + e, t8[e]);
+        } else
         if (tid >= CP0)
             for (int e = tid - CP0; e < total4; e += NTT - CP0) g4[e] = t4[e];
     }
@@ -307,7 +342,7 @@
                 const unsigned long long key = wave_sort_first<16>(lane < TPB ? wg_keys[0][0][lane] : KEY_SENTINEL, lane);
                 if (lane < ra.K) {
                     if (ra.part_k) {
-                        ra.part_k[(size_t)lane * n_wg + wg] = key;
+                        st_wt<LAST>(ra.part_k + ((size_t)lane * n_wg + wg), key);
                     } else {
                         ra.part_c[(size_t)wg * ra.K + lane] = key_cost(key);
                         ra.part_i[(size_t)wg * ra.K + lane] = key_idx(key);
@@ -331,7 +366,7 @@
                     const bool filler = (mine >> 32) == (KEY_SENTINEL >> 32) && (unsigned)mine >= KEY_FILL_LO;
                     const unsigned long long key = filler ? KEY_SENTINEL : mine;
                     if (ra.part_k) {
-                        ra.part_k[(size_t)place * n_wg + wg] = key;
+                        st_wt<LAST>(ra.part_k + ((size_t)place * n_wg + wg), key);
                     } else {
                         ra.part_c[(size_t)wg * ra.K + place] = key_cost(key);
                         ra.part_i[(size_t)wg * ra.K + place] = key_idx(key);
@@ -346,15 +381,39 @@
             if (ra.dbg && tid == 0 && wg == 0) ra.dbg[12] = wall_clock64();
         }
         if (ra.dbg && tid == 0 && wg == 0) ra.dbg[13] = wall_clock64();
-        if (ra.K > 0 && wg < n_wg) wg_merge_emit<RW>(wg_keys, run_key, ra.K, lane, wave, ra, wg, n_wg);
+        if (ra.K > 0 && wg < n_wg) wg_merge_emit<RW, LAST>(wg_keys, run_key, ra.K, lane, wave, ra, wg, n_wg);
     }
     if (ra.dbg && tid == 0 && wg == 0) ra.dbg[14] = wall_clock64();
+    if constexpr (LAST) {
+        asm volatile("s_waitcnt vmcnt(0)" ::: "memory");
+        __syncthreads();
+        if (tid == 0) my_ticket = __hip_atomic_fetch_add(lp->ticket, 1u, __ATOMIC_RELAXED, __HIP_MEMORY_SCOPE_AGENT);
+        __syncthreads();
+        const int ticket = (int)my_ticket;
+        __builtin_amdgcn_fence(__ATOMIC_ACQUIRE, "wavefront");
+        if (ticket != lp->n_tickets - 1) {
+            if (lp->noise_form == 2) {
+                const int per = (lp->z1.n + lp->n_tickets - 2) / (lp->n_tickets - 1);
+                const int r0 = ticket * per;
+                draw_rows(lp->z1, r0 < lp->z1.n ? r0 : lp->z1.n, r0 + per < lp->z1.n ? r0 + per : lp->z1.n);
+                if (ticket == 0) draw_rows(lp->z2, 0, lp->z2.n);
+            }
+            return;
+        }
+        if (tid == 0) __hip_atomic_store(lp->ticket, 0u, __ATOMIC_RELAXED, __HIP_MEMORY_SCOPE_AGENT);
+        merge_single_body<12, false, true>(lp->fin, ms, sel, cand, slot, tid < MERGE_WG);
+    }
 }
 
 
 template <int H, int D, int O, int KIND, int ROUNDS, int RW, int KREG, bool REC, int ARITH>
 __global__ __launch_bounds__(sr_threads(D, RW) + (KREG > 0 ? 64 : 0)) void sample_rollout_kernel(FastIterArgs a) {
     sample_rollout_body<H, D, O, KIND, ROUNDS, RW, KREG, REC, ARITH>(a.s, a.r, a.m, a.p);
+}
+
+template <int H, int D, int O, int KIND, int ROUNDS, int RW, int KREG, bool REC, int ARITH>
+__global__ __launch_bounds__(sr_threads(D, RW) + (KREG > 0 ? 64 : 0)) void ticket_sample_rollout_kernel(FastLastArgs a) {
+    sample_rollout_body<H, D, O, KIND, ROUNDS, RW, KREG, REC, ARITH, true>(a.it.s, a.it.r, a.it.m, a.it.p, &a.l);
 }
 
 template <int H, int D, int O, int KIND, int ROUNDS, int RW, int KREG, int ARITH>
@@ -439,6 +498,9 @@
     static void solo(int grid, hipStream_t st, const FastIterArgs& a) {
         hipLaunchKernelGGL((sample_rollout_kernel<H, D, O, KIND, 10, RW, KREG, REC, ARITH>), dim3(grid), dim3(THREADS), 0, st, a);
     }
+    static void last(int grid, hipStream_t st, const FastLastArgs& a) {
+        if constexpr (!REC) hipLaunchKernelGGL((ticket_sample_rollout_kernel<H, D, O, KIND, 10, RW, KREG, REC, ARITH>), dim3(grid), dim3(THREADS), 0, st, a);
+    }
     static void batch(int grid, int n, hipStream_t st, const FastIterArgs* args_dev, const BatchBases& bases) {
         hipLaunchKernelGGL((sample_rollout_batch_kernel<H, D, O, KIND, 10, RW, KREG, ARITH>), dim3(grid, n), dim3(THREADS), 0, st, args_dev, bases);
     }
@@ -487,6 +549,34 @@
            [&] { sample_rollout_dispatch(k, [&](auto inst) { inst.solo(k.wgs[0] + k.wgs[1], cx.st, a); }); });
 }
 
+static bool last_key(const BatchHint& bh, int h, int d, int O, int kind, int arith, int n_rows, bool merge_prologue, LaunchKey& k) {
+    if (bh.mult > 1 || !sample_rollout_shape(bh, h, d, O, 10, n_rows, 0, &k.wgs[0], &k.waves)) return false;
+    k.family = LAUNCH_SAMPLE_ROLLOUT;
+    k.h = h, k.d = d, k.O = O, k.kind = kind, k.arith = arith;
+    k.form = merge_prologue ? 1 : 0;
+    return true;
+}
+bool sample_rollout_last_ok(const BatchHint& bh, int h, int d, int O, int kind, int arith, int rounds, int n_rows, int K, bool merge_prologue) {
+    LaunchKey k;
+    if (rounds != 10 || K + 1 > 12 || !last_key(bh, h, d, O, kind, arith, n_rows, merge_prologue, k)) return false;
+    return sample_rollout_dispatch(k, [](auto) {});
+}
+void launch_sample_rollout_last(const LaunchCtx& cx, FastLastArgs& a, int h, int d, int O, int kind, bool merge_prologue) {
+    LaunchKey k;
+    if (!last_key(cx.hint, h, d, O, kind, a.it.r.arith, a.it.r.n_rows, merge_prologue, k)) return;
+    LastMergeArgs& l = a.l;
+    l.n_tickets = k.wgs[0];
+    l.wgs1 = l.wgs2 = 0;
+    if (l.z1.n <= 0) l.noise_form = 0;
+    if (l.noise_form == 2 && l.n_tickets < 2) l.noise_form = 1;
+    if (l.noise_form == 1) {
+        const int tpb = 16 * k.waves;
+        l.wgs1 = (l.z1.n + tpb - 1) / tpb;
+        l.wgs2 = l.z2.n > 0 ? (l.z2.n + tpb - 1) / tpb : 0;
+    }
+    sample_rollout_dispatch(k, [&](auto inst) { inst.last(k.wgs[0] + l.wgs1 + l.wgs2, cx.st, a); });
+}
+
 void launch_sample_rollout_batch(const LaunchKey& k, const FastIterArgs* args_dev, const BatchBases& bases, int n, hipStream_t st) {
     sample_rollout_dispatch(k, [&](auto inst) {
         if constexpr (decltype(inst)::BATCHED) inst.batch(k.wgs[0], n, st, args_dev, bases);
diff --git a/icem_amd/csrc/k_merge.hip b/icem_amd/csrc/k_merge.hip
--- a/icem_amd/csrc/k_merge.hip
+++ b/icem_amd/csrc/k_merge.hip
@@ -1,116 +1,28 @@
 #include "fused_dev.h"
+#include "merge_body.h"
 #include "refit.h"
 
 namespace icem {
 
 namespace {
-
-template <int KREG, bool REC>
-__device__ __forceinline__ void merge_single_body(const MergeSingleArgs& a, unsigned char* smem_raw) {
-    __shared__ unsigned long long sel[64];
-    __shared__ unsigned long long cand[64];
-    __shared__ int slot[64];
-    typedef float __attribute__((address_space(3))) * LdsF;
-    const LdsF new_mean = (LdsF)smem_raw;
-    const int tid = threadIdx.x;
-    const int lane = tid & 63;
-    const int hd = a.h * a.d;
-    if (a.dbg && threadIdx.x == 0) a.dbg[0] = wall_clock64();
-    constexpr int EPL = 4;
-    const bool pre = hd <= MERGE_WG * EPL;
-    float om[EPL], os[EPL], blo[EPL], bhi[EPL];
-#pragma unroll
-    for (int i = 0; i < EPL; ++i) {
-        const int e = tid + i * MERGE_WG;
-        om[i] = (pre && e < hd) ? a.mean[e] : 0.f;
-        os[i] = (pre && e < hd) ? a.std[e] : 0.f;
-    }
-    auto request_bounds = [&]() {
-#pragma unroll
-        for (int i = 0; i < EPL; ++i) {
-            const int e = tid + i * MERGE_WG;
-            blo[i] = (pre && a.last && e < hd) ? a.low[e % a.d] : 0.f;
-            bhi[i] = (pre && a.last && e < hd) ? a.high[e % a.d] : 0.f;
-        }
-    };
-    if (REC || tid >= 64) request_bounds();
-    if constexpr (REC) {
-        merge_select_records_wg(a, tid < 64, lane, tid, MERGE_WG, sel, slot);
-        if (a.dbg && threadIdx.x == 0) a.dbg[4] = wall_clock64();
-    } else {
-        if (tid < 64) merge_select_shallow<3>(a, lane, cand, sel);
-        if (a.dbg && threadIdx.x == 0) a.dbg[4] = wall_clock64();
-        if (tid < 64) request_bounds();
-        __syncthreads();
-    }
-    const float* rows[KREG];
-    merge_rows<KREG, REC>(a, sel, slot, rows);
-    float best0 = 0.f;
-    auto finish_one = [&](int e, float old_mean, float old_std) {
-        float xs[KREG];
-#pragma unroll
-        for (int r = 0; r < KREG; ++r) xs[r] = rows[r][e];
-#pragma unroll
-        for (int r = 0; r < KREG; ++r) asm volatile("" : "+v"(xs[r]));
-        float nm, ns;
-        refit_element_regs<float, KREG>(a.K, a.alpha, old_mean, old_std, xs, nm, ns);
-#pragma unroll
-        for (int r = 0; r < KREG; ++r)
-            if (r < a.K) a.elites_next[(size_t)r * hd + e] = xs[r];
-        if (!a.last) {
-            a.mean_out[e] = nm;
-            a.std_out[e] = ns;
-        } else {
-            new_mean[e] = nm;
-        }
-        if (e == tid) best0 = xs[0];
-    };
-    if (pre) {
-#pragma unroll
-        for (int i = 0; i < EPL; ++i) {
-            const int e = tid + i * MERGE_WG;
-            if (e < hd) finish_one(e, om[i], os[i]);
-        }
-    } else {
-        for (int e = tid; e < hd; e += MERGE_WG) finish_one(e, a.mean[e], a.std[e]);
-    }
-    if (a.dbg && threadIdx.x == 0) a.dbg[5] = wall_clock64();
-    if (tid < a.K) a.elites_cost_next[tid] = key_cost(sel[tid]);
-    if (a.last) {
-        __syncthreads();
-        if (pre) {
-#pragma unroll
-            for (int i = 0; i < EPL; ++i) {
-                const int e = tid + i * MERGE_WG;
-                if (e < hd) {
-                    a.mean_out[e] = (e + a.d < hd) ? new_mean[e + a.d] : new_mean[e];
-                    a.std_out[e] = (bhi[i] - blo[i]) / 2.f * a.init_std;
-                }
-            }
-        } else {
-            for (int e = tid; e < hd; e += MERGE_WG) {
-                const int j = e % a.d;
-                a.mean_out[e] = (e + a.d < hd) ? new_mean[e + a.d] : new_mean[e];
-                a.std_out[e] = (a.high[j] - a.low[j]) / 2.f * a.init_std;
-            }
-        }
-        if (tid < a.d) a.executed[tid] = best0;
-        if (tid == 0) a.best_cost[0] = key_cost(sel[0]);
-    }
-    if (a.dbg && threadIdx.x == 0) a.dbg[6] = wall_clock64();
-}
 
 template <int KREG, bool REC>
 __global__ __launch_bounds__(MERGE_WG) void merge_single_kernel(MergeSingleArgs a) {
     extern __shared__ __attribute__((aligned(16))) unsigned char smem_raw[];
-    merge_single_body<KREG, REC>(a, smem_raw);
+    __shared__ unsigned long long sel[64];
+    __shared__ unsigned long long cand[64];
+    __shared__ int slot[64];
+    merge_single_body<KREG, REC>(a, smem_raw, sel, cand, slot);
 }
 
 template <int H, int KREG>
 __global__ __launch_bounds__(MERGE_WG) void merge_noise_kernel(MergeSingleArgs a, FastSampleArgs z1, FastSampleArgs z2, int wgs1) {
     extern __shared__ __attribute__((aligned(16))) unsigned char smem_raw[];
+    __shared__ unsigned long long sel[64];
+    __shared__ unsigned long long cand[64];
+    __shared__ int slot[64];
     if (blockIdx.x == 0) {
-        merge_single_body<KREG, false>(a, smem_raw);
+        merge_single_body<KREG, false>(a, smem_raw, sel, cand, slot);
         return;
     }
     const bool second = (int)blockIdx.x > wgs1;
@@ -142,9 +54,12 @@
 __global__ __launch_bounds__(MERGE_WG) void merge_noise_batch_kernel(const MergeNoiseBatchArgs* __restrict__ args, BatchBases bases, int wgs1) {
     extern __shared__ __attribute__((aligned(16))) unsigned char smem_raw[];
     const MergeNoiseBatchArgs& g = args[blockIdx.y];
+    __shared__ unsigned long long sel[64];
+    __shared__ unsigned long long cand[64];
+    __shared__ int slot[64];
     if (blockIdx.x == 0) {
         const MergeSingleArgs a = from_device(g.a);
-        merge_single_body<KREG, false>(a, smem_raw);
+        merge_single_body<KREG, false>(a, smem_raw, sel, cand, slot);
         return;
     }
     const bool second = (int)blockIdx.x > wgs1;
@@ -199,7 +114,8 @@
     __syncthreads();
     pack_records_body<KREG>(pk, n_loc, shard_lo, records, px, reinterpret_cast<float*>(smem_raw), sel, tid, MERGE_WG);
     __syncthreads();
-    merge_single_body<KREG, true>(m, smem_raw);
+    __shared__ int slot[64];
+    merge_single_body<KREG, true>(m, smem_raw, sel, cand, slot);
 }
 
 __global__ __launch_bounds__(1024) void topk_small_kernel(const float* costs, int n, int K, float* out_c, int* out_i) {
diff --git a/icem_amd/csrc/merge_body.h b/icem_amd/csrc/merge_body.h
--- /dev/null
+++ b/icem_amd/csrc/merge_body.h
@@ -0,0 +1,100 @@
+#pragma once
+#include "fused_dev.h"
+#include "refit.h"
+
+namespace icem {
+
+template <int KREG, bool REC, bool AG = false>
+__device__ __forceinline__ void merge_single_body(const MergeSingleArgs& a, void* smem_raw, unsigned long long* sel, unsigned long long* cand,
+                                                  int* slot, bool active = true) {
+    typedef float __attribute__((address_space(3))) * LdsF;
+    const LdsF new_mean = (LdsF)smem_raw;
+    const int tid = threadIdx.x;
+    const int lane = tid & 63;
+    const int hd = active ? a.h * a.d : 0;
+    if (a.dbg && threadIdx.x == 0) a.dbg[0] = wall_clock64();
+    constexpr int EPL = 4;
+    const bool pre = hd <= MERGE_WG * EPL;
+    float om[EPL], os[EPL], blo[EPL], bhi[EPL];
+#pragma unroll
+    for (int i = 0; i < EPL; ++i) {
+        const int e = tid + i * MERGE_WG;
+        om[i] = (pre && e < hd) ? ld_ag<AG>(a.mean + e) : 0.f;
+        os[i] = (pre && e < hd) ? ld_ag<AG>(a.std + e) : 0.f;
+    }
+    auto request_bounds = [&]() {
+#pragma unroll
+        for (int i = 0; i < EPL; ++i) {
+            const int e = tid + i * MERGE_WG;
+            blo[i] = (pre && a.last && e < hd) ? a.low[e % a.d] : 0.f;
+            bhi[i] = (pre && a.last && e < hd) ? a.high[e % a.d] : 0.f;
+        }
+    };
+    if (REC || tid >= 64) request_bounds();
+    if constexpr (REC) {
+        merge_select_records_wg(a, tid < 64, lane, tid, MERGE_WG, sel, slot);
+        if (a.dbg && threadIdx.x == 0) a.dbg[4] = wall_clock64();
+    } else {
+        if (tid < 64) merge_select_shallow<3, AG>(a, lane, cand, sel);
+        if (a.dbg && threadIdx.x == 0) a.dbg[4] = wall_clock64();
+        if (tid < 64) request_bounds();
+        __syncthreads();
+    }
+    const float* rows[KREG];
+    merge_rows<KREG, REC>(a, sel, slot, rows);
+    float best0 = 0.f;
+    auto finish_one = [&](int e, float old_mean, float old_std) {
+        float xs[KREG];
+#pragma unroll
+        for (int r = 0; r < KREG; ++r) xs[r] = ld_ag<AG>(rows[r] + e);
+#pragma unroll
+        for (int r = 0; r < KREG; ++r) asm volatile("" : "+v"(xs[r]));
+        float nm, ns;
+        refit_element_regs<float, KREG>(a.K, a.alpha, old_mean, old_std, xs, nm, ns);
+#pragma unroll
+        for (int r = 0; r < KREG; ++r)
+            if (r < a.K) a.elites_next[(size_t)r * hd + e] = xs[r];
+        if (!a.last) {
+            a.mean_out[e] = nm;
+            a.std_out[e] = ns;
+        } else {
+            new_mean[e] = nm;
+        }
+        if (e == tid) best0 = xs[0];
+    };
+    if (pre) {
+#pragma unroll
+        for (int i = 0; i < EPL; ++i) {
+            const int e = tid + i * MERGE_WG;
+            if (e < hd) finish_one(e, om[i], os[i]);
+        }
+    } else {
+        for (int e = tid; e < hd; e += MERGE_WG) finish_one(e, ld_ag<AG>(a.mean + e), ld_ag<AG>(a.std + e));
+    }
+    if (a.dbg && threadIdx.x == 0) a.dbg[5] = wall_clock64();
+    if (active && tid < a.K) a.elites_cost_next[tid] = key_cost(sel[tid]);
+    if (a.last) {
+        __syncthreads();
+        if (pre) {
+#pragma unroll
+            for (int i = 0; i < EPL; ++i) {
+                const int e = tid + i * MERGE_WG;
+                if (e < hd) {
+                    a.mean_out[e] = (e + a.d < hd) ? new_mean[e + a.d] : new_mean[e];
+                    a.std_out[e] = (bhi[i] - blo[i]) / 2.f * a.init_std;
+                }
+            }
+        } else {
+            for (int e = tid; e < hd; e += MERGE_WG) {
+                const int j = e % a.d;
+                a.mean_out[e] = (e + a.d < hd) ? new_mean[e + a.d] : new_mean[e];
+                a.std_out[e] = (a.high[j] - a.low[j]) / 2.f * a.init_std;
+            }
+        }
+        if (active && tid < a.d) a.executed[tid] = best0;
+        if (tid == 0) a.best_cost[0] = key_cost(sel[0]);
+    }
+    if (a.dbg && threadIdx.x == 0) a.dbg[6] = wall_clock64();
+}
+
+}
diff --git a/icem_amd/csrc/options.h b/icem_amd/csrc/options.h
--- a/icem_amd/csrc/options.h
+++ b/icem_amd/csrc/options.h
@@ -16,6 +16,7 @@
     X(AHEAD_TAIL_FRAC, "ahead_tail_frac", 0.4)                                                                             \
     X(AHEAD_NEXT1_FRAC, "ahead_next1_frac", 0.3)                                                                           \
     X(AHEAD_NOISE_LDS_KB, "ahead_noise_lds_kb", -1.0)                                                                      \
+    X(LAST_MERGE_TICKET, "last_merge_ticket", 1.0)    \
     X(PREDRAW, "predraw", 1.0)                              \
     X(GK_SAMPLE, "gk_sample", 1.0)                          \
     X(GK_ROLLOUT_THREAD, "gk_rollout_thread", 0.0)                   \
diff --git a/icem_amd/csrc/plan.hip b/icem_amd/csrc/plan.hip
--- a/icem_amd/csrc/plan.hip
+++ b/icem_amd/csrc/plan.hip
@@ -604,7 +604,35 @@
                 fa.r = fast_rollout_args(h, n_rows, n_cand, K, b->obs0, actions, b->costs, pc, pi);
                 fa.r.part_k = (unsigned long long*)b->workspace;
                 fa.r.list_wgs = tail_rows > 0 ? one : 0;
-                {
+                const bool fused_last = last && h->ride.last_armed && c.world == 1 && !cx.rec && tail_rows == 0 && h->ticket_dev &&
+                                        sample_rollout_last_ok(cx.hint, c.horizon, c.act_dim, h->Of, h->model_kind, fa.r.arith, c.rng_rounds, n_rows, K, prologue);
+                h->ride.last_armed = false;
+                if (fused_last) {
+                    FastLastArgs la = zeroed_args<FastLastArgs>();
+                    la.it = fa;
+                    h->local.lists = one;
+                    const MergeArgsV a = merge_args<T>(h, b, mpc_step, it, MergeRoute{false, h->ride.last_mean_out, h->ride.last_std_out});
+                    MergeSingleArgs& m = la.l.fin;
+                    m.keep_base = -1;
+                    fill_single(m, a);
+                    m.n_lists = one;
+                    m.n_pool = h->pop[it] + shift_rows(h, mpc_step, it, false);
+                    m.part_k = (const unsigned long long*)b->workspace;
+                    m.actions = (const float*)b->actions;
+                    la.l.ticket = h->ticket_dev;
+                    if (it > 0 || fa.s.raw_src == nullptr) predraw_next_step(h, b, mpc_step, cx);
+                    if (h->ahead.tail_pending) {
+                        la.l.z1 = h->ahead.tail_args;
+                        la.l.z2 = h->ahead.tail2_args;
+                        la.l.noise_form = opt_i(OPT_LAST_MERGE_TICKET) == 2 ? 2 : 1;
+                        h->ahead.tail_pending = false;
+                    }
+                    {
+                        ProfScope prof(h, ICEM_K_SAMPLE_ROLLOUT, (long long)n_rows * c.horizon, st);
+                        launch_sample_rollout_last(cx, la, c.horizon, c.act_dim, h->Of, h->model_kind, prologue);
+                    }
+                    h->ride.last_done = true;
+                } else {
                     ProfScope prof(h, ICEM_K_SAMPLE_ROLLOUT, (long long)n_rows * c.horizon, st);
                     launch_sample_rollout(cx, fa, c.horizon, c.act_dim, h->Of, h->model_kind, prologue);
                 }
@@ -1294,9 +1322,19 @@
             bb.mean = cur_mean;
             bb.std = cur_std;
         }
+        const bool last = it == iters - 1;
+        h->ride.last_done = false;
+        h->ride.last_armed = last && opt_i(OPT_LAST_MERGE_TICKET) != 0 && c.dtype == ICEM_F32 && b->z_r == nullptr && h->use_fast && !cx.rec &&
+                             h->dbg == nullptr && !h->ride.pack_pending;
+        h->ride.last_mean_out = (float*)b->mean;
+        h->ride.last_std_out = (float*)b->std;
         rc = ICEM_DISPATCH(h, plan_iter_local_t<float>(h, &bb, mpc_step, it, cx), plan_iter_local_t<double>(h, &bb, mpc_step, it, cx));
         if (rc) return rc;
-        const bool last = it == iters - 1;
+        h->ride.last_armed = false;
+        if (h->ride.last_done) {
+            h->ride.last_done = false;
+            break;
+        }
         if (last) predraw_next_step(h, b, mpc_step, cx);
         bool fold = false;
         if (pingpong && !last && h->local.lists > 0) fold = prologue_possible(h, cx.hint, h->pop[it + 1]);
diff --git a/icem_amd/planner.py b/icem_amd/planner.py
--- a/icem_amd/planner.py
+++ b/icem_amd/planner.py
@@ -304,6 +304,11 @@
     def nonfinite_costs(self) -> int:
         n = C.c_int64()
         L.check(self.lib.icem_nonfinite_costs(self._h, C.byref(n), self._stream()))
+        return int(n.value)
+
+    def last_merge_ticket(self) -> int:
+        n = C.c_int64()
+        L.check(self.lib.icem_last_merge_ticket(self._h, C.byref(n), self._stream()))
         return int(n.value)
 
     F64_ARITH = {"chain": 0, "mfma": 1}
diff --git a/include/icem_hip.h b/include/icem_hip.h
--- a/include/icem_hip.h
+++ b/include/icem_hip.h
@@ -235,6 +235,7 @@
 int icem_f64_arith(const icem_handle* h);
 
 int icem_nonfinite_costs(icem_handle* h, int64_t* count_out, void* stream);
+int icem_last_merge_ticket(icem_handle* h, int64_t* count_out, void* stream);
 
 int icem_set_option(const char* name, double value);
 int icem_get_option(const char* name, double* value_out);
```

Measured after the change: 7.365 billion. -3.9%, worse.
